# TomClabault/RayTracerCPP

Measured on NVIDIA B200. Metric: Mrays/s (primary+shadow), higher is better.
Workload: dtype f32

## Files before the change

### include/rtb200.h

```cpp
#ifndef RTB200_H
#define RTB200_H

#include <stddef.h>
#include <stdint.h>

#ifdef __cplusplus
extern "C" {
#endif

typedef struct RtContext RtContext;

typedef enum RtStatus {
    RT_OK = 0,
    RT_ERR_INVALID = -1,
    RT_ERR_CUDA = -2,
    RT_ERR_STATE = -3,
    RT_ERR_UNSUPPORTED = -4
} RtStatus;

typedef struct RtMaterial {
    float ambient_coeff[3];
    float diffuse[3];
    float specular[3];
    float emission[3];
// ... 44 lines not shown
    float ssao_amount;
    int32_t enable_clipping;
} RtSettings;

enum {
    RT_TEX_AO = 0,
    RT_TEX_DIFFUSE = 1,
    RT_TEX_NORMAL = 2,
    RT_TEX_ROUGHNESS = 3,
    RT_TEX_SKYSPHERE = 4,
    RT_TEX_SKYBOX_RIGHT = 5,
    RT_TEX_SKYBOX_LEFT = 6,
    RT_TEX_SKYBOX_TOP = 7,
    RT_TEX_SKYBOX_BOTTOM = 8,
    RT_TEX_SKYBOX_BACK = 9,
    RT_TEX_SKYBOX_FRONT = 10,
    RT_TEX_DISPLACEMENT = 11,
    RT_TEX_COUNT = 12
};

typedef struct RtRenderStats {
    uint64_t primary_rays;
    uint64_t shadow_rays;
    uint64_t reflection_rays;
    uint64_t reflection_shadow_rays;
    uint64_t primary_hits;
    uint32_t kernel_launches;
    float    device_ms;
    float    trace_primary_ms;
    float    shade_ms;
    float    reflect_ms;
    float    compact_ms;
    float    resolve_ms;
    uint64_t primary_volume_tests, primary_triangle_tests;
    uint64_t shadow_volume_tests, shadow_triangle_tests;
    uint64_t reflection_volume_tests, reflection_triangle_tests;
    uint64_t traced_primary_rays;
    uint64_t primary_fetched_bytes, shadow_fetched_bytes, reflection_fetched_bytes;
} RtRenderStats;

typedef struct RtBvhInfo {
    uint64_t triangles;
    uint64_t nodes;
    uint64_t leaves;
    uint64_t empty_leaves;
    uint64_t interior;
    uint32_t max_depth_reached;
    uint32_t max_leaf_size;
    uint64_t child_records;
    uint64_t device_bytes;
    double   build_ms;
    double   upload_ms;
} RtBvhInfo;

void rt_default_settings(RtSettings* s);
uint32_t rt_pixel_seed(uint32_t pixel_index, uint32_t rng_seed);

int rt_create(int device, RtContext** out);
void rt_destroy(RtContext* ctx);
const char* rt_last_error(const RtContext* ctx);

enum {
    RT_OPT_COUNT_WORK = 0,
    RT_OPT_CHUNK_PIXELS = 1,
    RT_OPT_REFILL_PRIMARY = 3,
    RT_OPT_REFILL_SHADE = 4,
    RT_OPT_TRI_BATCH = 5,
    RT_OPT_PACKETS = 6,
    RT_OPT_PACKET_ROUNDS = 7,
    RT_OPT_PRIMARY_ROUNDS = 11,
    RT_OPT_ITEM_ROUNDS = 10,
    RT_OPT_ITEM_PASSES = 16,
    RT_OPT_FUSED_ITEMS = 12,
    RT_OPT_TOP_TABLE = 13,
    RT_OPT_DEVICE_BUILD = 15,
    RT_OPT_SHADOW_SORT = 14,
    RT_OPT_SCREEN_CULL = 8,
    RT_OPT_LANES = 9,
    RT_OPT_PACKET_CULL = 19,
    RT_OPT_FAN_LANES = 20,
    RT_OPT_GRAPH = 18,
    RT_OPT_RASTER_UNITS = 17,
    RT_OPT_LIGHT_CULL = 21,
    RT_OPT_LEAF_SPLIT = 2
};
int rt_set_option(RtContext* ctx, int option, int64_t value);
int rt_set_host_threads(int n);
int rt_set_stream(RtContext* ctx, void* cuda_stream);

int rt_set_triangles(RtContext* ctx, const float* xyz9, const float* uv6, const int32_t* mat, size_t n);

int rt_build_bvh(RtContext* ctx, int max_depth, int leaf_max_obj_count);
int rt_bvh_info(const RtContext* ctx, RtBvhInfo* out);

int rt_transform_triangles(RtContext* ctx, const float m[16], int max_depth, int leaf_max_obj_count);

typedef struct RtObjMesh RtObjMesh;
int rt_obj_load(const char* path, const float transform[16], int32_t current_material_count, RtObjMesh** out, char* err, size_t err_cap);
void rt_obj_free(RtObjMesh* mesh);
size_t rt_obj_triangle_count(const RtObjMesh* mesh);
size_t rt_obj_material_count(const RtObjMesh* mesh);
const float* rt_obj_xyz9(const RtObjMesh* mesh);
const float* rt_obj_uv6(const RtObjMesh* mesh);
const int32_t* rt_obj_material_indices(const RtObjMesh* mesh);
const RtMaterial* rt_obj_materials(const RtObjMesh* mesh);
const char* rt_obj_material_name(const RtObjMesh* mesh, size_t i);
void rt_precompute_materials(RtMaterial* mats, size_t n);

int rt_set_materials(RtContext* ctx, const RtMaterial* mats, size_t n);

int rt_add_sphere(RtContext* ctx, const float center[3], float radius, int32_t mat_index);
int rt_add_plane(RtContext* ctx, const float point[3], const float normal[3], int32_t mat_index);
int rt_clear_analytic_shapes(RtContext* ctx);

int rt_set_texture_f32(RtContext* ctx, int slot, const float* rgba, int width, int height);
int rt_set_texture_u8(RtContext* ctx, int slot, const uint8_t* rgba, int width, int height);
int rt_clear_texture(RtContext* ctx, int slot);

int rt_set_camera(RtContext* ctx, const float proj_inv[16], const float cam_to_world[16], const float position[3]);
void rt_perspective_inverse(float fov, float aspect, float znear, float zfar, float proj_inv_out[16]);
void rt_invert_transform(const float m[16], float out[16]);
void rt_transform_point(const float m[16], const float p[3], float out[3]);

int rt_set_projection(RtContext* ctx, float fov, float aspect, float znear, float zfar);

int rt_set_light(RtContext* ctx, const float position[3]);

int rt_render(RtContext* ctx, const RtSettings* settings, uint32_t* argb_out, RtRenderStats* stats);

int rt_render_device(RtContext* ctx, const RtSettings* settings, uint32_t* d_argb_out,
                     int tile_size, int tile_mod, int tile_rem, RtRenderStats* stats);

int rt_render_device_begin(RtContext* ctx, const RtSettings* settings, uint32_t* d_argb_out,
                           int tile_size, int tile_mod, int tile_rem);
int rt_render_device_end(RtContext* ctx, RtRenderStats* stats);

#define RT_FRAME_HANDLE_BYTES 64
int rt_frame_alloc(RtContext* ctx, size_t bytes, void** d_ptr_out, unsigned char handle_out[RT_FRAME_HANDLE_BYTES]);
int rt_frame_open(RtContext* ctx, const unsigned char handle[RT_FRAME_HANDLE_BYTES], void** d_ptr_out);
int rt_frame_close(RtContext* ctx, void* d_ptr);
int rt_frame_free(RtContext* ctx, void* d_ptr);

int rt_frame_to_host(RtContext* ctx, const uint32_t* d_frame, uint32_t* host_out, size_t n_pixels);

int rt_tile_count(const RtSettings* settings, int tile_size, int tile_mod, int tile_rem);
int rt_pack_tiles(RtContext* ctx, const RtSettings* settings, const uint32_t* d_frame, uint32_t* d_staging,
                  int tile_size, int tile_mod, int tile_rem);
int rt_unpack_tiles(RtContext* ctx, const RtSettings* settings, uint32_t* d_frame, const uint32_t* d_staging,
                    int tile_size, int tile_mod, int tile_rem);

int rt_unpack_gathered(RtContext* ctx, const RtSettings* settings, uint32_t* d_frame, const uint32_t* d_gathered,
                       int tile_size, int tile_mod, int self_rem);

int rt_intersect(RtContext* ctx, const float* o3, const float* d3, size_t n,
                 int32_t* tri_id, float* t, float* u, float* v);

int rt_occluded(RtContext* ctx, const float* p3, const float* n3, size_t n, uint8_t* occluded);

int rt_generate_primary_rays(RtContext* ctx, const RtSettings* settings, float* o3, float* d3);

int rt_resolve_ssaa(RtContext* ctx, const uint32_t* argb_in, int width, int height, int factor, uint32_t* argb_out);

#ifdef __cplusplus
}
#endif
#endif
// ... 1 lines not shown
```

### raytracercpp_b200/api.py

```python
from __future__ import annotations

import ctypes as C
from pathlib import Path

import numpy as np

PKG = Path(__file__).resolve().parent
LIB_PATH = PKG / "librtb200.so"

RT_OK, RT_ERR_INVALID, RT_ERR_CUDA, RT_ERR_STATE, RT_ERR_UNSUPPORTED = 0, -1, -2, -3, -4
RT_SHADING, RT_ABS_NORMALS_SHADING, RT_PASTEL_NORMALS_SHADING, RT_BARYCENTRIC_COORDINATES_SHADING, RT_VISUALIZE_AO = range(5)
RT_TEX_AO, RT_TEX_DIFFUSE, RT_TEX_NORMAL, RT_TEX_ROUGHNESS, RT_TEX_SKYSPHERE = range(5)
RT_TEX_SKYBOX_RIGHT, RT_TEX_SKYBOX_LEFT, RT_TEX_SKYBOX_TOP, RT_TEX_SKYBOX_BOTTOM, RT_TEX_SKYBOX_BACK, RT_TEX_SKYBOX_FRONT = range(5, 11)
RT_TEX_DISPLACEMENT = 11
RT_OPT_COUNT_WORK, RT_OPT_CHUNK_PIXELS, RT_OPT_LEAF_SPLIT, RT_OPT_REFILL_PRIMARY, RT_OPT_REFILL_SHADE, RT_OPT_TRI_BATCH, RT_OPT_PACKETS = 0, 1, 2, 3, 4, 5, 6
RT_OPT_PACKET_ROUNDS, RT_OPT_SCREEN_CULL, RT_OPT_LANES, RT_OPT_ITEM_ROUNDS, RT_OPT_PRIMARY_ROUNDS, RT_OPT_FUSED_ITEMS, RT_OPT_TOP_TABLE, RT_OPT_SHADOW_SORT, RT_OPT_DEVICE_BUILD, RT_OPT_ITEM_PASSES = 7, 8, 9, 10, 11, 12, 13, 14, 15, 16
RT_OPT_RASTER_UNITS, RT_OPT_GRAPH, RT_OPT_PACKET_CULL, RT_OPT_FAN_LANES, RT_OPT_LIGHT_CULL = 17, 18, 19, 20, 21


class RtError(RuntimeError):
    def __init__(self, code: int, message: str):
        super().__init__(f"rtb200 error {code}: {message}")
        self.code = code
        self.message = message


class RtMaterial(C.Structure):
    _fields_ = [("ambient_coeff", C.c_float * 3), ("diffuse", C.c_float * 3), ("specular", C.c_float * 3),
                ("emission", C.c_float * 3), ("reflection", C.c_float), ("roughness", C.c_float), ("ns", C.c_float),
                ("specular_threshold", C.c_float)]


SETTINGS_FIELDS = [
    "image_width", "image_height", "enable_ssaa", "ssaa_factor", "hybrid_rasterization_tracing", "shading_method",
    "compute_shadows", "max_recursion_depth", "enable_bvh", "bvh_max_depth", "bvh_leaf_object_count", "enable_ssao",
    "enable_ambient", "enable_diffuse", "enable_specular", "enable_emissive", "rough_reflections_sample_count",
    "enable_ao_mapping", "enable_diffuse_mapping", "enable_normal_mapping", "enable_displacement_mapping",
    "enable_roughness_mapping", "enable_skysphere", "enable_skybox",
]


class RtSettings(C.Structure):
    _fields_ = [(n, C.c_int32) for n in SETTINGS_FIELDS] + [("rng_seed", C.c_uint32), ("displacement_mapping_strength", C.c_float),
                                                              ("parallax_mapping_steps", C.c_int32),
                                                              ("ssao_sample_count", C.c_int32), ("ssao_radius", C.c_float), ("ssao_amount", C.c_float),
                                                             ("enable_clipping", C.c_int32)]

    def copy(self) -> "RtSettings":
        out = RtSettings()
        C.memmove(C.byref(out), C.byref(self), C.sizeof(RtSettings))
        return out


class RtRenderStats(C.Structure):
    _fields_ = [("primary_rays", C.c_uint64), ("shadow_rays", C.c_uint64), ("reflection_rays", C.c_uint64),
                ("reflection_shadow_rays", C.c_uint64), ("primary_hits", C.c_uint64), ("kernel_launches", C.c_uint32),
                ("device_ms", C.c_float), ("trace_primary_ms", C.c_float), ("shade_ms", C.c_float),
                ("reflect_ms", C.c_float), ("compact_ms", C.c_float), ("resolve_ms", C.c_float),
                ("primary_volume_tests", C.c_uint64), ("primary_triangle_tests", C.c_uint64),
                ("shadow_volume_tests", C.c_uint64), ("shadow_triangle_tests", C.c_uint64),
                ("reflection_volume_tests", C.c_uint64), ("reflection_triangle_tests", C.c_uint64),
                ("traced_primary_rays", C.c_uint64), ("primary_fetched_bytes", C.c_uint64), ("shadow_fetched_bytes", C.c_uint64),
                ("reflection_fetched_bytes", C.c_uint64)]

    def as_dict(self) -> dict:
        return {n: getattr(self, n) for n, _ in self._fields_}

    @property
    def total_rays(self) -> int:
        return self.primary_rays + self.shadow_rays + self.reflection_rays + self.reflection_shadow_rays

    @property
    def traced_rays(self) -> int:
        return self.traced_primary_rays + self.shadow_rays + self.reflection_rays + self.reflection_shadow_rays

    @property
    def work_bytes(self) -> int:
        v = self.primary_volume_tests + self.shadow_volume_tests + self.reflection_volume_tests
        t = self.primary_triangle_tests + self.shadow_triangle_tests + self.reflection_triangle_tests
        return 56 * v + 36 * t


class RtBvhInfo(C.Structure):
    _fields_ = [("triangles", C.c_uint64), ("nodes", C.c_uint64), ("leaves", C.c_uint64), ("empty_leaves", C.c_uint64),
                ("interior", C.c_uint64), ("max_depth_reached", C.c_uint32), ("max_leaf_size", C.c_uint32),
                ("child_records", C.c_uint64), ("device_bytes", C.c_uint64), ("build_ms", C.c_double),
                ("upload_ms", C.c_double)]

    def as_dict(self) -> dict:
        return {n: getattr(self, n) for n, _ in self._fields_}


FP, IP, UP, BP = C.POINTER(C.c_float), C.POINTER(C.c_int32), C.POINTER(C.c_uint32), C.POINTER(C.c_uint8)

ABI = {
    "rt_default_settings": (None, [C.POINTER(RtSettings)]),
    "rt_pixel_seed": (C.c_uint32, [C.c_uint32, C.c_uint32]),
    "rt_create": (C.c_int, [C.c_int, C.POINTER(C.c_void_p)]),
    "rt_destroy": (None, [C.c_void_p]),
    "rt_last_error": (C.c_char_p, [C.c_void_p]),
# ... 315 lines not shown
```

### raytracercpp_b200/build.py

```python
from __future__ import annotations

import os
import shutil
import subprocess
import sys
from pathlib import Path

PKG = Path(__file__).resolve().parent
CSRC = PKG / "csrc"
LIB = PKG / "librtb200.so"
SOURCES = [CSRC / "rtb200.cu", CSRC / "octree_build.cpp", CSRC / "scene_io.cpp"]
HEADERS = [CSRC / "kernels.cuh", CSRC / "octree_device.cuh", CSRC / "light_cull.cuh", CSRC / "host_common.h", CSRC / "rt_device.h", CSRC / "rt_math.h", CSRC / "scene_layout.h",
           CSRC / "ssao.cuh", CSRC / "ssao_device.h", CSRC / "raster.cuh", CSRC / "raster_device.h",
           PKG.parent / "include" / "rtb200.h"]

NVCC_FLAGS = [
    "-gencode", "arch=compute_100a,code=sm_100a",
    "-O3", "-lineinfo", "-std=c++17",
    "--fmad=false", "--prec-div=true", "--prec-sqrt=true",
    "-Xcompiler", "-fPIC,-fopenmp,-ffp-contract=off,-O3",
    "-ccbin", "/usr/bin/g++",
    "-shared", "-lgomp",
]


def nvcc() -> str:
    for cand in (os.environ.get("NVCC"), shutil.which("nvcc"), "/usr/local/cuda/bin/nvcc"):
        if cand and Path(cand).exists():
            return cand
    raise RuntimeError("nvcc not found")


def up_to_date() -> bool:
    if not LIB.exists():
        return False
    t = LIB.stat().st_mtime
    return all(p.stat().st_mtime <= t for p in SOURCES + HEADERS + [Path(__file__)])


def build(force: bool = False, verbose: bool = False, extra=(), out: Path | None = None) -> Path:
    if out is None and not force and up_to_date():
        return LIB
    cmd = [nvcc(), *NVCC_FLAGS, *extra, "-o", str(out or LIB), *map(str, SOURCES)]
    if verbose:
        print(" ".join(cmd), flush=True)
    res = subprocess.run(cmd, capture_output=True, text=True)
    if verbose or res.returncode:
        sys.stderr.write(res.stdout + res.stderr)
    if res.returncode:
        raise RuntimeError("nvcc failed")
    return out or LIB


if __name__ == "__main__":
    argv = sys.argv[1:]
    out = Path(argv[argv.index("--out") + 1]) if "--out" in argv else None
    extra = [a for a in argv if a.startswith("-D")] + (["-Xptxas", "-v"] if "--ptxas" in argv else [])
    print(build(force="--force" in argv, verbose=True, extra=extra, out=out))
```

### raytracercpp_b200/csrc/kernels.cuh

```cuda
#pragma once

#include <cuda_runtime.h>
#include "rt_device.h"

namespace rtb {

constexpr int kPatch = 8;
constexpr int kPrimaryThreads = 128;
constexpr int kQueueThreads = 128;
constexpr int kPrimaryFetch = 1;
constexpr int kStepsPerCheck = 4;
constexpr unsigned kParkCtas = 296;
constexpr unsigned kFusedGenerations = 12;
constexpr int kItemPasses = 6;
#ifndef RTB_SHADE_MINB
#define RTB_SHADE_MINB 7
#endif

constexpr int kSubQueues = 32;
struct alignas(128) SubQueue {
    unsigned int n;
    unsigned int next;
    unsigned int pad[30];
};
struct alignas(16) FusedTotals {
    unsigned int reserved;
    unsigned int done;
    unsigned int packets_done;
    unsigned int pad;
};

struct ChunkCounters {
    unsigned int next_patch;
    unsigned int next_shade;
    unsigned int n_hits;
    unsigned int n_refl;
    unsigned int stack_overflow;
    unsigned int n_split;
    unsigned int items_n[kItemPasses];
    unsigned int items_next[kItemPasses];
    unsigned int p_split, p_items_n[kItemPasses], p_items_next[kItemPasses];
    SubQueue sq[2][kSubQueues];
    FusedTotals ft[2];
    unsigned long long refl_rays;
    unsigned long long refl_shadow_rays;
    unsigned long long primary_vol, primary_tri, shadow_vol, shadow_tri, refl_vol, refl_tri;
    unsigned long long primary_fetch, shadow_fetch, refl_fetch;
    unsigned long long traced_primary;
    unsigned int rounds_hist[2][16];
    unsigned int max_rounds[2];
    unsigned long long max_packet_ns[2], sum_packet_ns[2];
};

RT_DEV unsigned long long global_ns()
{
    unsigned long long t;
    asm volatile("mov.u64 %0, %%globaltimer;" : "=l"(t));
    return t;
}

RT_DEV void note_packet(ChunkCounters* cnt, int which, unsigned rounds, unsigned long long ns)
{
    const int b = rounds ? min(31 - __clz(rounds), 15) : 0;
    atomicAdd(&cnt->rounds_hist[which][b], 1u);
    atomicMax(&cnt->max_rounds[which], rounds);
    atomicMax(&cnt->max_packet_ns[which], ns);
    atomicAdd(&cnt->sum_packet_ns[which], ns);
}

RT_DEV void flush_work(TraceCounters& tc, unsigned long long* vol, unsigned long long* tri, unsigned long long* fetch)
{
    unsigned long long v = tc.vol_tests, t = tc.tri_tests, f = 64ull * tc.rec_fetch + 48ull * tc.tri_fetch;
#pragma unroll
    for (int o = 16; o > 0; o >>= 1) {
        v += __shfl_xor_sync(0xffffffffu, v, o);
        t += __shfl_xor_sync(0xffffffffu, t, o);
        f += __shfl_xor_sync(0xffffffffu, f, o);
    }
    if ((threadIdx.x & 31u) == 0) {
        if (v) atomicAdd(vol, v);
        if (t) atomicAdd(tri, t);
        if (f) atomicAdd(fetch, f);
    }
}

struct WorkView {
    const uint32_t* tiles;
    uint32_t tile_begin, tile_end;
    int32_t tiles_x;
    int32_t tile_px;
    int32_t patches_per_side;
    const uint32_t* cover;
    int32_t cover_words;
};

struct QueueView {
    int32_t* slot_tri;
    float* slot_t;
    float* slot_u;
    float* slot_v;
    uint32_t* hit_slot;
    uint32_t* hit_sorted;
    uint32_t sort_mode, sort_slots;
    float* g_z;
    V3* g_n;
    uint32_t* split_base;
    uint32_t* split_active;
    uint32_t* split_occ;
    uint4* items;
    uint32_t split_capacity, item_capacity;
    uint32_t* item_ready;
    uint32_t* split_pending;
    uint32_t tag;
    unsigned long long* split_best;
    uint32_t* refl_idx;
    float* refl_rgb;
    unsigned long long* refl_cnt;
    uint32_t capacity;
};

RT_DEV bool slot_pixel(const WorkView& wk, const FrameView& fr, uint32_t slot, int& px, int& py)
{
    const uint32_t pps = (uint32_t)wk.patches_per_side;
    const uint32_t per_tile = pps * pps * (uint32_t)(kPatch * kPatch);
    const uint32_t tile = wk.tiles[wk.tile_begin + slot / per_tile];
    const uint32_t in_tile = slot % per_tile;
    const uint32_t patch = in_tile / (uint32_t)(kPatch * kPatch), in_patch = in_tile % (uint32_t)(kPatch * kPatch);
    const int lx = (int)(patch % pps) * kPatch + (int)(in_patch & 7u);
    const int ly = (int)(patch / pps) * kPatch + (int)(in_patch >> 3);
    px = (int)(tile % (uint32_t)wk.tiles_x) * wk.tile_px + lx;
    py = (int)(tile / (uint32_t)wk.tiles_x) * wk.tile_px + ly;
    return lx < wk.tile_px && ly < wk.tile_px && px < fr.rw && py < fr.rh;
}

RT_DEV bool covered(const WorkView& wk, int px, int py)
{
    if (wk.cover == nullptr) return true;
    const uint32_t w = __ldg(wk.cover + ((uint32_t)py >> 2) * (uint32_t)wk.cover_words + ((uint32_t)px >> 8));
    return ((w >> (((uint32_t)px >> 3) & 31u)) & 1u) != 0u;
}

struct Tuning {
    int32_t primary_refill;
    int32_t shade_refill;
    int32_t tri_batch;
    int32_t packets;
    int32_t packet_rounds;
    int32_t item_rounds;
    int32_t primary_rounds;
    int32_t fused;
    int32_t packet_min, item_min, primary_min;
    int32_t item_passes;
    int32_t cull;
};

struct Drain {
    const unsigned int* counter;
    uint32_t total;
    int min_rounds;
};
RT_DEV Drain no_drain() { Drain d; d.counter = nullptr; d.total = 0u; d.min_rounds = 0; return d; }
RT_DEV Drain make_drain(const unsigned int* counter, uint32_t total, int min_rounds)
{
    Drain d; d.counter = min_rounds > 0 ? counter : nullptr; d.total = total; d.min_rounds = min_rounds; return d;
}

template <bool ANY, bool COUNT>
RT_DEV void warp_step(const SceneView& sc, RayState& S, RayStack& K, TraceCounters* tc, bool alive, const Tuning& tune)
{
    const unsigned want_c = __ballot_sync(0xffffffffu, alive && S.mode == RT_MODE_CHILDREN);
    const unsigned want_t = __ballot_sync(0xffffffffu, alive && S.mode == RT_MODE_TRIANGLES);
    if (want_c != 0u && __popc(want_t) < tune.tri_batch) {
        if (alive && S.mode == RT_MODE_CHILDREN) ray_child_step<COUNT>(sc, S, K, tc);
    } else if (want_t != 0u) {
        if (alive && S.mode == RT_MODE_TRIANGLES) ray_triangle_step<ANY, COUNT>(sc, S, K, tc);
    }
}
// ... 141 lines not shown
    const float2 q1b = *(reinterpret_cast<const float2*>(rec + 1) + 1);
    const float4 q2 = rec[2], q3 = rec[3];
    RT_SLAB(3, q1b.x, q1b.y)
    RT_SLAB(4, q2.x, q2.y)
    RT_SLAB(5, q2.z, q2.w)
    RT_SLAB(6, q3.x, q3.y)
#undef RT_SLAB
    link = f4_bits(q3.z); meta = f4_bits(q3.w);
    const bool ok = pass && (tn <= tf + 2.0f * sr.slack) && (tf + sr.slack >= 0.0f) && (tn - sr.slack <= t_limit);
    return ok ? tn - sr.slack : INFINITY;
}

RT_DEV uint32_t ld_vol(const unsigned int* p) { return *((const volatile unsigned int*)p); }

template <bool ORDERED, bool COUNT>
RT_DEV bool packet_cell(const float4* rec, uint32_t count, const SlabRay& sr, float t_max, bool active, PacketStack& K, int& sp, TraceCounters& tc,
                        uint32_t keep)
{
    const unsigned lane = threadIdx.x & 31u;
    const int base = sp;
    for (uint32_t m = keep; m != 0u; m &= m - 1u) {
        const uint32_t k = (uint32_t)__ffs((int)m) - 1u;
        if (COUNT && active) tc.vol_tests++;
        uint32_t cl = 0u, cm = 0u;
        const float tn = slab_entry_packet<ORDERED>(rec + 4 * k, sr, t_max, active, cl, cm);
        if (__ballot_sync(0xffffffffu, tn != INFINITY) == 0u) continue;
        const float tmin = warp_min(tn);
        if (sp >= RT_STACK_SIZE) return false;
        if (lane == 0) {
            int j = sp;
            while (j > base && K.t[j - 1] < tmin) {
                K.t[j] = K.t[j - 1]; K.link[j] = K.link[j - 1]; K.meta[j] = K.meta[j - 1];
                --j;
            }
            K.t[j] = tmin; K.link[j] = cl; K.meta[j] = cm;
        }
        ++sp;
    }
    return true;
}

struct TopTable {
    float4 rec[4 * RT_TOP_RECORDS];
    unsigned long long bar;
};
struct NoTopTable {
    unsigned long long bar;
};
template <bool TOP> struct TopStorage { typedef TopTable type; };
template <> struct TopStorage<false> { typedef NoTopTable type; };
RT_DEV const float4* top_pointer(TopTable& T) { return T.rec; }
RT_DEV const float4* top_pointer(NoTopTable&) { return nullptr; }
RT_DEV void load_top_table(const SceneView&, NoTopTable&) {}

RT_DEV void load_top_table(const SceneView& sc, TopTable& T)
{
    const uint32_t bar = (uint32_t)__cvta_generic_to_shared(&T.bar), dst = (uint32_t)__cvta_generic_to_shared(&T.rec[0]);
    const uint32_t bytes = (uint32_t)sc.top_n * 64u;
    if (bytes == 0u) return;
    if (threadIdx.x == 0) {
        asm volatile("mbarrier.init.shared::cta.b64 [%0], 1;" ::"r"(bar));
        asm volatile("fence.mbarrier_init.release.cluster;" ::: "memory");
    }
    __syncthreads();
    if (threadIdx.x == 0) {
        asm volatile("mbarrier.arrive.expect_tx.shared::cta.b64 _, [%0], %1;" ::"r"(bar), "r"(bytes) : "memory");
        asm volatile("cp.async.bulk.shared::cluster.global.mbarrier::complete_tx::bytes [%0], [%1], %2, [%3];" ::"r"(dst), "l"(sc.top), "r"(bytes), "r"(bar)
                     : "memory");
    }
    asm volatile(
        "{\n"
        ".reg .pred p;\n"
        "TOP_WAIT:\n"
        "mbarrier.try_wait.parity.shared::cta.b64 p, [%0], 0;\n"
        "@!p bra TOP_WAIT;\n"
        "}\n" ::"r"(bar)
        : "memory");
}

template <bool ANY, bool COUNT, bool CULL = false>
RT_DEV bool packet_trace(const SceneView& sc, PacketStack& K, const float4* top, bool& active, V3 o, V3 d, float t_max, V3 p, float dist2,
                         HitRec& best, bool& occluded, TraceCounters& tc, unsigned& overflow, int max_rounds, unsigned& rounds,
                         uint32_t start_link = 0u, uint32_t start_meta = 0u, int32_t best_orig = 0x7fffffff,
                         const unsigned int* poll_occ = nullptr, const unsigned long long* poll_best = nullptr, Drain drain = no_drain())
{
    const unsigned lane = threadIdx.x & 31u;
    SlabRay sr;
    slab_setup(o, d, sr);
    const V3 md = -d;
    best.tri = -1; best.t = -1.0f; best.u = 1.0f; best.v = 0.0f;
    occluded = false;
    unsigned neg_mask = 0u;
#ifdef RTB_NO_ORDERED
    bool ordered = false;
#else
    bool ordered = true;
#endif
#pragma unroll
    for (int i = 0; i < 7; i++) {
        const bool nz = active && sr.inv[i] != 0.0f;
        const unsigned bn = __ballot_sync(0xffffffffu, nz && sr.inv[i] < 0.0f), bp = __ballot_sync(0xffffffffu, nz && sr.inv[i] > 0.0f);
        if (bn != 0u && bp != 0u) ordered = false;
        if (bn != 0u) neg_mask |= 1u << i;
    }
    const unsigned f = lane & 3u;
    const bool swap_lo = ordered && ((neg_mask >> (2u * f)) & 1u) != 0u;
    const bool swap_hi = ordered && f < 3u && ((neg_mask >> (2u * f + 1u)) & 1u) != 0u;
    uint32_t link = start_link, meta = start_meta;
    if (start_meta == 0u) {
        const rt_f4* r = sc.recs;
        rt_f4 q0 = RT_LDG4(r), q1 = RT_LDG4(r + 1), q2 = RT_LDG4(r + 2), q3 = RT_LDG4(r + 3);
        if (COUNT && active) tc.vol_tests++;
        if (COUNT && lane == 0) tc.rec_fetch++;
        const float tn = active ? slab_entry(q0, q1, q2, q3, sr, t_max) : INFINITY;
        link = f4_bits(q3.z); meta = f4_bits(q3.w);
        if (__ballot_sync(0xffffffffu, tn != INFINITY) == 0u || (meta & ~(RT_LEAF_BIT | RT_META_TOP)) == 0u) return true;
        if (ANY && (__ldg(sc.blk_occ) & 1u) == 0u) return true;
    }
    int sp = 0;
    for (;;) {
        if (max_rounds > 0 && sp < RT_STACK_SIZE) {
            bool stop = (int)rounds >= max_rounds;
            if (!stop && drain.counter != nullptr && (int)rounds >= drain.min_rounds && (rounds & 15u) == 0u) {
                uint32_t handed = 0;
                if (lane == 0) handed = ld_vol(drain.counter);
                stop = __shfl_sync(0xffffffffu, handed, 0) >= drain.total;
            }
            if (stop) {
                if (lane == 0) { K.t[sp] = 0.0f; K.link[sp] = link; K.meta[sp] = meta; K.saved = sp + 1; }
                __syncwarp();
                return false;
            }
        }
        ++rounds;
        if ((rounds & 3u) == 0u) {
            if (ANY && poll_occ != nullptr) {
                uint32_t w = 0;
                if (lane == 0) w = ld_vol(poll_occ);
                w = __shfl_sync(0xffffffffu, w, 0);
                if ((w >> lane) & 1u) active = false;
                if (__ballot_sync(0xffffffffu, active) == 0u) return true;
            }
            if (!ANY && poll_best != nullptr) {
                const unsigned long long key = *((const volatile unsigned long long*)(poll_best + lane));
                if (key != ~0ull) {
                    const float te = __uint_as_float((uint32_t)(key >> 32));
                    const int32_t oe = (int32_t)(uint32_t)key;
                    if (te < t_max || (te == t_max && oe < best_orig)) { t_max = te; best_orig = oe; }
                }
            }
        }
        if (!(meta & RT_LEAF_BIT)) {
            const uint32_t count = meta & RT_META_COUNT_MASK;
            const bool in_top = top != nullptr && (meta & RT_META_TOP) != 0u;
            if (lane < 4u * count) {
                float4 v = in_top ? top[4u * ((meta >> RT_META_TOP_SHIFT) & 0xffu) + lane] : RT_LDG4(sc.recs + 4 * (size_t)link + lane);
                if (swap_lo) { const float t = v.x; v.x = v.y; v.y = t; }
                if (swap_hi) { const float t = v.z; v.z = v.w; v.w = t; }
                K.stage[lane] = v;
            }
            if (COUNT && lane == 0 && !in_top) tc.rec_fetch += count;
            __syncwarp();
            uint32_t keep = (1u << count) - 1u;
            if (ANY) keep &= __ldg(sc.blk_occ + (link >> 1));
            if (CULL) {
                const uint32_t child = lane >> 2;
                const float4 pl = K.plane[lane & 3u];
                const float4 b0 = K.stage[4u * child];
                const float2 b1 = *reinterpret_cast<const float2*>(&K.stage[4u * child + 1u]);
                const float ax = pl.x * (pl.x > 0.0f ? fmaxf(b0.x, b0.y) : fminf(b0.x, b0.y));
                const float ay = pl.y * (pl.y > 0.0f ? fmaxf(b0.z, b0.w) : fminf(b0.z, b0.w));
                const float az = pl.z * (pl.z > 0.0f ? fmaxf(b1.x, b1.y) : fminf(b1.x, b1.y));
                const bool outside = (ax + ay + az) - pl.w < -4.0e-6f * (fabsf(ax) + fabsf(ay) + fabsf(az) + fabsf(pl.w));
                unsigned m = __ballot_sync(0xffffffffu, outside);
                m |= m >> 1;
                m |= m >> 2;
                unsigned in = ~m & 0x11111111u;
                in = (in | (in >> 3)) & 0x03030303u;
                in = (in | (in >> 6)) & 0x000f000fu;
                in = (in | (in >> 12)) & 0xffu;
                keep &= in;
            }
            const bool fits = ordered ? packet_cell<true, COUNT>(K.stage, count, sr, t_max, active, K, sp, tc, keep)
                                      : packet_cell<false, COUNT>(K.stage, count, sr, t_max, active, K, sp, tc, keep);
            if (!fits) { overflow = 1u; return true; }
            __syncwarp();
        } else {
            const uint32_t cnt = meta & ~RT_LEAF_BIT;
            const uint32_t per_round = CULL ? 8u : 10u;
            for (uint32_t first = 0; first < cnt; first += per_round) {
                const uint32_t m = min(per_round, cnt - first);
                uint32_t keep = (1u << m) - 1u;
                if (ANY) {
                    const uint32_t at = link + first;
                    keep &= __funnelshift_r(__ldg(sc.tri_occ + (at >> 5)), __ldg(sc.tri_occ + (at >> 5) + 1), at & 31u);
                    if (keep == 0u) continue;
                }
                if (lane < 3u * m) K.stage[lane] = RT_LDG4(sc.tris + 3 * (size_t)(link + first) + lane);
                if (COUNT && lane == 0) tc.tri_fetch += m;
                __syncwarp();
                if (CULL) {
                    const uint32_t tri = lane >> 2;
                    const float4 pl = K.plane[lane & 3u];
                    const float4 va = K.stage[3u * tri], vb = K.stage[3u * tri + 1u], vc = K.stage[3u * tri + 2u];
                    const float da = (pl.x * va.x + pl.y * va.y + pl.z * va.z) - pl.w;
                    const float db = (pl.x * vb.x + pl.y * vb.y + pl.z * vb.z) - pl.w;
                    const float dc = (pl.x * vc.x + pl.y * vc.y + pl.z * vc.z) - pl.w;
                    const float mag = fabsf(pl.w) + fmaxf(fabsf(va.x), fmaxf(fabsf(vb.x), fabsf(vc.x))) + fmaxf(fabsf(va.y), fmaxf(fabsf(vb.y), fabsf(vc.y))) +
                                      fmaxf(fabsf(va.z), fmaxf(fabsf(vb.z), fabsf(vc.z)));
                    const bool outside = fmaxf(da, fmaxf(db, dc)) < -4.0e-6f * mag;
                    unsigned om = __ballot_sync(0xffffffffu, outside);
                    om |= om >> 1;
                    om |= om >> 2;
                    unsigned in = ~om & 0x11111111u;
                    in = (in | (in >> 3)) & 0x03030303u;
                    in = (in | (in >> 6)) & 0x000f000fu;
                    in = (in | (in >> 12)) & 0xffu;
                    keep &= in;
                }
                for (uint32_t km = keep; km != 0u; km &= km - 1u) {
                    const uint32_t i = (uint32_t)__ffs((int)km) - 1u;
                    const float4 p0 = K.stage[3 * i], p1 = K.stage[3 * i + 1], p2 = K.stage[3 * i + 2];
                    if (COUNT && active) tc.tri_tests++;
                    float t, u, v;
                    if (active && tri_test(p0, p1, p2, o, md, t, u, v)) {
                        const uint32_t tri = link + first + i;
                        if (ANY) {
                            if (t > 0.0f) {
                                V3 q = o + t * d;
                                if (length2(p - q) < dist2) { occluded = true; active = false; }
                            }
                        } else if (t < t_max || (t == t_max && sc.orig[tri] < best_orig)) {
                            t_max = t;
                            best_orig = sc.orig[tri];
                            best.tri = (int32_t)tri; best.t = t; best.u = u; best.v = v;
                        }
                    }
                }
                __syncwarp();
            }
            if (ANY && __ballot_sync(0xffffffffu, active) == 0u) return true;
        }
        bool got = false;
        while (sp > 0) {
            --sp;
            const float et = K.t[sp];
            if (__ballot_sync(0xffffffffu, active && et <= t_max) == 0u) continue;
            link = K.link[sp]; meta = K.meta[sp];
            got = true;
            break;
        }
        if (!got) return true;
    }
}

RT_DEV bool emit_items(const QueueView& q, unsigned int* items_n, const PacketStack& K, int pass, uint32_t sidx)
{
    const unsigned lane = threadIdx.x & 31u;
    const uint32_t n = (uint32_t)K.saved;
    uint32_t at = 0;
    if (lane == 0) at = atomicAdd(&items_n[pass], n);
    at = __shfl_sync(0xffffffffu, at, 0);
    const bool ok = at + n <= q.item_capacity;
    uint4* region = q.items + (size_t)pass * q.item_capacity;
    for (uint32_t i = lane; i < n && at + i < q.item_capacity; i += 32u)
        region[at + i] = ok ? make_uint4(sidx, K.link[i], K.meta[i], 0u) : make_uint4(0xffffffffu, 0u, 0u, 0u);
    __syncwarp();
    return ok;
}

RT_DEV unsigned long long closest_key(float t, int32_t orig) { return ((unsigned long long)__float_as_uint(t) << 32) | (uint32_t)orig; }
constexpr unsigned long long kNoHitKey = ~0ull;

#ifndef RTB_PRIMARY_MINB
#define RTB_PRIMARY_MINB 8
#endif
#define RTB_PRIMARY_BOUNDS __launch_bounds__(kPrimaryThreads, RTB_PRIMARY_MINB)
template <bool COUNT, bool TOP>
__global__ void RTB_PRIMARY_BOUNDS
k_primary_packet(SceneView sc, FrameView fr, WorkView wk, QueueView q, ChunkCounters* cnt, uint32_t* super, Tuning tune)
{
    __shared__ PacketStack stacks[kPrimaryThreads / 32];
    PacketStack& K = stacks[threadIdx.x >> 5];
    __shared__ typename TopStorage<TOP>::type top_table;
    load_top_table(sc, top_table);
    const float4* top = top_pointer(top_table);
    const unsigned lane = threadIdx.x & 31u;
    const uint32_t pps = (uint32_t)wk.patches_per_side;
    const uint32_t total = (wk.tile_end - wk.tile_begin) * pps * pps * (uint32_t)(kPatch * kPatch);
    TraceCounters tc = zero_counters();
    unsigned overflow = 0;
    uint32_t traced = 0;
    uint32_t nxt = 0;
    if (lane == 0) nxt = atomicAdd(&cnt->next_patch, 32u * kPrimaryFetch);
    for (;;) {
        const uint32_t first = __shfl_sync(0xffffffffu, nxt, 0);
        if (first >= total) break;
        if (lane == 0) nxt = atomicAdd(&cnt->next_patch, 32u * kPrimaryFetch);
#pragma unroll 1
        for (uint32_t b = 0; b < (uint32_t)kPrimaryFetch; b++) {
            const uint32_t base = first + 32u * b;
            if (base >= total) break;
            const uint32_t slot = base + lane;
            int px = 0, py = 0;
            const bool active = slot < total && slot_pixel(wk, fr, slot, px, py);
            V3 o = v3(0, 0, 0), d = v3(0, 0, 1);
            const bool inside = active && covered(wk, px, py);
            if (__ballot_sync(0xffffffffu, inside) == 0u) {
                if (slot < total) {
                    q.slot_tri[slot] = -1;
                    if (active) {
                        if (miss_needs_ray(fr)) primary_ray(fr, px, py, o, d);
                        super[(size_t)py * fr.rw + px] = quantise_argb(shade_miss(sc, fr, d));
                    }
                }
                continue;
            }
            if (active) primary_ray(fr, px, py, o, d);
            traced += (uint32_t)__popc(__ballot_sync(0xffffffffu, active));
            HitRec best;
            bool occ, live = active;
            unsigned rounds = 0;
            const unsigned long long t0 = COUNT ? global_ns() : 0ull;
            if (!((tune.cull & 1) != 0 && packet_set_cull(K, active, o, o + d, 0.0f))) packet_no_cull(K);
            const bool finished = packet_trace<false, COUNT, true>(sc, K, top, live, o, d, INFINITY, o, 0.0f, best, occ, tc, overflow, tune.primary_rounds, rounds,
                                                                   0u, 0u, 0x7fffffff, nullptr, nullptr, make_drain(&cnt->next_patch, total, tune.primary_min));
            __syncwarp();
            if (COUNT && lane == 0) note_packet(cnt, 0, rounds, global_ns() - t0);
            if (!finished) {
                const unsigned am = __ballot_sync(0xffffffffu, active);
                uint32_t sidx = 0;
                if (lane == 0) sidx = atomicAdd(&cnt->p_split, 1u);
                sidx = __shfl_sync(0xffffffffu, sidx, 0);
                if (sidx < q.split_capacity && emit_items(q, cnt->p_items_n, K, 0, sidx)) {
                    if (lane == 0) { q.split_base[sidx] = base; q.split_active[sidx] = am; }
                    q.split_best[(size_t)sidx * 32u + lane] = (active && best.tri >= 0) ? closest_key(best.t, sc.orig[best.tri]) : kNoHitKey;
                    continue;
                }
                if (sidx < q.split_capacity && lane == 0) { q.split_base[sidx] = base; q.split_active[sidx] = 0u; }
                live = active;
                packet_trace<false, COUNT>(sc, K, top, live, o, d, INFINITY, o, 0.0f, best, occ, tc, overflow, 0, rounds);
                __syncwarp();
            }
            if (slot < total) {
                const bool hit = active && best.tri >= 0 && best.t > 0.1f;
                q.slot_tri[slot] = hit ? best.tri : -1;
                if (hit) { q.slot_t[slot] = best.t; q.slot_u[slot] = best.u; q.slot_v[slot] = best.v; }
                else if (active) {
                    if (sc.n_shapes > 0) q.slot_t[slot] = (best.tri >= 0 && best.t > 0.0f) ? best.t : -1.0f;
                    super[(size_t)py * fr.rw + px] = quantise_argb(shade_miss(sc, fr, d));
                }
            }
        }
    }
    if (overflow) atomicOr(&cnt->stack_overflow, 1u);
    if (lane == 0 && traced) atomicAdd(&cnt->traced_primary, (unsigned long long)traced);
    if (COUNT) flush_work(tc, &cnt->primary_vol, &cnt->primary_tri, &cnt->primary_fetch);
}

template <bool COUNT>
__global__ void RTB_PRIMARY_BOUNDS
k_primary_items(SceneView sc, FrameView fr, WorkView wk, QueueView q, ChunkCounters* cnt, Tuning tune, int pass)
{
    __shared__ PacketStack stacks[kPrimaryThreads / 32];
    PacketStack& K = stacks[threadIdx.x >> 5];
    const float4* top = nullptr;
    const unsigned lane = threadIdx.x & 31u;
    const uint32_t n = min(cnt->p_items_n[pass], q.item_capacity);
    const uint4* region = q.items + (size_t)pass * q.item_capacity;
    const int budget = pass + 1 < tune.item_passes ? tune.item_rounds : 0;
    TraceCounters tc = zero_counters();
    unsigned overflow = 0;
    for (;;) {
        uint32_t i = 0;
        if (lane == 0) i = atomicAdd(&cnt->p_items_next[pass], 1u);
        i = __shfl_sync(0xffffffffu, i, 0);
        if (i >= n) break;
        const uint4 item = region[i];
        const uint32_t sidx = item.x;
        if (sidx == 0xffffffffu) continue;
        const uint32_t base = q.split_base[sidx];
        const uint32_t slot = base + lane;
        const bool active = ((q.split_active[sidx] >> lane) & 1u) != 0u;
        int px = 0, py = 0;
        V3 o = v3(0, 0, 0), d = v3(0, 0, 1);
        if (active) { slot_pixel(wk, fr, slot, px, py); primary_ray(fr, px, py, o, d); }
        unsigned long long* mine = q.split_best + (size_t)sidx * 32u + lane;
        const unsigned long long seen = *((volatile unsigned long long*)mine);
        const float t_start = seen == kNoHitKey ? INFINITY : __uint_as_float((uint32_t)(seen >> 32));
        const int32_t orig_start = seen == kNoHitKey ? 0x7fffffff : (int32_t)(uint32_t)seen;
        HitRec best;
        bool occ, live = active;
        unsigned rounds = 0;
        if (!((tune.cull & 1) != 0 && packet_set_cull(K, active, o, o + d, 0.0f))) packet_no_cull(K);
        bool finished = packet_trace<false, COUNT, true>(sc, K, top, live, o, d, t_start, o, 0.0f, best, occ, tc, overflow, budget, rounds, item.y, item.z, orig_start,
                                                         nullptr, nullptr, make_drain(&cnt->p_items_next[pass], n, tune.item_min));
        __syncwarp();
        if (active && best.tri >= 0) atomicMin(mine, closest_key(best.t, sc.orig[best.tri]));
        if (!finished && !emit_items(q, cnt->p_items_n, K, pass + 1, sidx)) {
            const unsigned long long now = *((volatile unsigned long long*)mine);
            const float t2 = now == kNoHitKey ? INFINITY : __uint_as_float((uint32_t)(now >> 32));
            const int32_t o2 = now == kNoHitKey ? 0x7fffffff : (int32_t)(uint32_t)now;
            live = active;
            packet_trace<false, COUNT>(sc, K, top, live, o, d, t2, o, 0.0f, best, occ, tc, overflow, 0, rounds, item.y, item.z, o2);
            __syncwarp();
            if (active && best.tri >= 0) atomicMin(mine, closest_key(best.t, sc.orig[best.tri]));
        }
    }
    if (overflow) atomicOr(&cnt->stack_overflow, 1u);
// ... 1027 lines not shown
    if (active && best.tri >= 0) atomicMin(mine, closest_key(best.t, sc.orig[best.tri]));
    if (!finished && !fq_emit(q, cnt, 0, K, sidx, item.w + 1u, false)) {
        const unsigned long long now = *((volatile unsigned long long*)mine);
        const float t2 = now == kNoHitKey ? INFINITY : __uint_as_float((uint32_t)(now >> 32));
        const int32_t o2 = now == kNoHitKey ? 0x7fffffff : (int32_t)(uint32_t)now;
        live = active;
        packet_trace<false, COUNT>(sc, K, top, live, o, d, t2, o, 0.0f, best, occ, tc, overflow, 0, rounds, item.y, item.z, o2, nullptr,
                                   q.split_best + (size_t)sidx * 32u);
        __syncwarp();
        if (active && best.tri >= 0) atomicMin(mine, closest_key(best.t, sc.orig[best.tri]));
    }
    __threadfence();
    __syncwarp();
    uint32_t left = 0;
    if (lane == 0) left = atomicSub(&q.split_pending[sidx], 1u);
    left = __shfl_sync(0xffffffffu, left, 0);
    if (left == 1u) {
        __threadfence();
        primary_finish_record(sc, fr, wk, q, super, sidx, total);
    }
    if (lane == 0) { __threadfence(); atomicAdd(&cnt->ft[0].done, 1u); }
}

template <bool COUNT>
__global__ void RTB_PRIMARY_BOUNDS
k_primary_fused(SceneView sc, FrameView fr, WorkView wk, QueueView q, ChunkCounters* cnt, uint32_t* super, Tuning tune)
{
    __shared__ PacketStack stacks[kPrimaryThreads / 32];
    PacketStack& K = stacks[threadIdx.x >> 5];
    const float4* top = nullptr;
    const unsigned lane = threadIdx.x & 31u;
    const uint32_t pps = (uint32_t)wk.patches_per_side;
    const uint32_t total = (wk.tile_end - wk.tile_begin) * pps * pps * (uint32_t)(kPatch * kPatch);
    const uint32_t total_packets = total >> 5;
    TraceCounters tc = zero_counters();
    unsigned overflow = 0;
    uint32_t traced = 0;
    uint32_t nxt = 0;
    if (lane == 0) nxt = atomicAdd(&cnt->next_patch, 32u);
    bool more = true;
    uint32_t my_packets = 0;
    unsigned backoff = 250u;
    const uint32_t per_round = 32u * gridDim.x * (kPrimaryThreads / 32);
    uint32_t rem = total / per_round;
    for (;;) {
        uint4 item;
        const int got = tune.primary_rounds > 0 ? fq_take(q, cnt, 0, !more, item) : 0;
        if (got == 1) {
            primary_item_fused<COUNT>(sc, fr, wk, q, cnt, super, fq_budget(tune.item_rounds, more ? rem : 0u), K, top, item, total, tc, overflow);
            backoff = 250u;
            continue;
        }
        if (!more) {
            if (got == 2) continue;
            if (tune.primary_rounds <= 0 || blockIdx.x >= kParkCtas) break;
            bool done = false;
            if (lane == 0) done = fq_all_done(&cnt->ft[0], total_packets);
            if (__shfl_sync(0xffffffffu, done ? 1 : 0, 0)) break;
            __nanosleep(backoff);
            backoff = min(backoff * 2u, 4000u);
            continue;
        }
        const uint32_t base = __shfl_sync(0xffffffffu, nxt, 0);
        if (base >= total) {
            more = false;
            if (lane == 0 && my_packets && tune.primary_rounds > 0) { __threadfence(); atomicAdd(&cnt->ft[0].packets_done, my_packets); }
            continue;
        }
        if (lane == 0) nxt = atomicAdd(&cnt->next_patch, 32u);
        rem = (total - base) / per_round;
        const uint32_t slot = base + lane;
        int px = 0, py = 0;
        const bool active = slot_pixel(wk, fr, slot, px, py);
        V3 o = v3(0, 0, 0), d = v3(0, 0, 1);
        const bool inside = active && covered(wk, px, py);
        bool deferred = false;
        if (__ballot_sync(0xffffffffu, inside) == 0u) {
            q.slot_tri[slot] = -1;
            if (active) {
                if (miss_needs_ray(fr)) primary_ray(fr, px, py, o, d);
                super[(size_t)py * fr.rw + px] = quantise_argb(shade_miss(sc, fr, d));
            }
        } else {
            if (active) primary_ray(fr, px, py, o, d);
            traced += (uint32_t)__popc(__ballot_sync(0xffffffffu, active));
            HitRec best;
            bool occ, live = active;
            unsigned rounds = 0;
            const unsigned long long t0 = COUNT ? global_ns() : 0ull;
            const bool finished = packet_trace<false, COUNT>(sc, K, top, live, o, d, INFINITY, o, 0.0f, best, occ, tc, overflow,
                                                             fq_budget(tune.primary_rounds, rem), rounds);
            __syncwarp();
            if (COUNT && lane == 0) note_packet(cnt, 0, rounds, global_ns() - t0);
            if (!finished) {
                const unsigned am = __ballot_sync(0xffffffffu, active);
                uint32_t sidx = 0xffffffffu;
                if (lane == 0) sidx = atomicAdd(&cnt->p_split, 1u);
                sidx = __shfl_sync(0xffffffffu, sidx, 0);
                if (sidx < q.split_capacity) {
                    if (lane == 0) { q.split_base[sidx] = base; q.split_active[sidx] = am; }
                    q.split_best[(size_t)sidx * 32u + lane] = (active && best.tri >= 0) ? closest_key(best.t, sc.orig[best.tri]) : kNoHitKey;
                    __threadfence();
                    __syncwarp();
                    deferred = fq_emit(q, cnt, 0, K, sidx, 0u, true);
                }
                if (!deferred) {
                    live = active;
                    packet_trace<false, COUNT>(sc, K, top, live, o, d, INFINITY, o, 0.0f, best, occ, tc, overflow, 0, rounds);
                    __syncwarp();
                }
            }
            if (!deferred) {
                const bool hit = active && best.tri >= 0 && best.t > 0.1f;
                q.slot_tri[slot] = hit ? best.tri : -1;
                if (hit) { q.slot_t[slot] = best.t; q.slot_u[slot] = best.u; q.slot_v[slot] = best.v; }
                else if (active) {
                    if (sc.n_shapes > 0) q.slot_t[slot] = (best.tri >= 0 && best.t > 0.0f) ? best.t : -1.0f;
                    super[(size_t)py * fr.rw + px] = quantise_argb(shade_miss(sc, fr, d));
                }
            }
        }
        ++my_packets;
    }
    if (overflow) atomicOr(&cnt->stack_overflow, 1u);
    if (lane == 0 && traced) atomicAdd(&cnt->traced_primary, (unsigned long long)traced);
    if (COUNT) flush_work(tc, &cnt->primary_vol, &cnt->primary_tri, &cnt->primary_fetch);
}

__global__ void k_fill_miss(SceneView sc, FrameView fr, WorkView wk, uint32_t* super)
{
    const uint32_t n_tiles = wk.tile_end - wk.tile_begin;
    const uint32_t background = quantise_argb(shade_miss(sc, fr, v3(0, 0, 1)));
    if (!miss_needs_ray(fr) && (wk.tile_px & 3) == 0 && (fr.rw & 3) == 0 && (reinterpret_cast<uintptr_t>(super) & 15u) == 0) {
        const uint32_t groups_per_row = (uint32_t)wk.tile_px >> 2;
        const uint32_t per_tile = groups_per_row * (uint32_t)wk.tile_px;
        const uint4 c4 = make_uint4(background, background, background, background);
        for (uint32_t t = blockIdx.x; t < n_tiles; t += gridDim.x) {
            const uint32_t tile = wk.tiles[wk.tile_begin + t];
            const int x0 = (int)(tile % (uint32_t)wk.tiles_x) * wk.tile_px, y0 = (int)(tile / (uint32_t)wk.tiles_x) * wk.tile_px;
            for (uint32_t g = threadIdx.x; g < per_tile; g += blockDim.x) {
                const int px = x0 + (int)((g % groups_per_row) << 2), py = y0 + (int)(g / groups_per_row);
                if (px < fr.rw && py < fr.rh) *reinterpret_cast<uint4*>(super + (size_t)py * fr.rw + px) = c4;
            }
        }
        return;
    }
    const uint32_t per_tile = (uint32_t)wk.tile_px * (uint32_t)wk.tile_px;
    for (uint32_t t = blockIdx.x; t < n_tiles; t += gridDim.x) {
        const uint32_t tile = wk.tiles[wk.tile_begin + t];
        const int x0 = (int)(tile % (uint32_t)wk.tiles_x) * wk.tile_px, y0 = (int)(tile / (uint32_t)wk.tiles_x) * wk.tile_px;
        for (uint32_t g = threadIdx.x; g < per_tile; g += blockDim.x) {
            const int px = x0 + (int)(g % (uint32_t)wk.tile_px), py = y0 + (int)(g / (uint32_t)wk.tile_px);
            if (px >= fr.rw || py >= fr.rh) continue;
            uint32_t c = background;
            if (miss_needs_ray(fr)) {
                V3 o, d;
                primary_ray(fr, px, py, o, d);
                c = quantise_argb(shade_miss(sc, fr, d));
            }
            super[(size_t)py * fr.rw + px] = c;
        }
    }
}

__global__ void k_resolve(const uint32_t* super, uint32_t* out, WorkView wk, int tile_size, int factor, int width, int height, uint32_t n_box,
                          uint32_t fill)
{
    const uint32_t per_tile = (uint32_t)tile_size * (uint32_t)tile_size;
    const uint64_t total = (uint64_t)(wk.tile_end - wk.tile_begin) * per_tile;
    for (uint64_t g = (uint64_t)blockIdx.x * blockDim.x + threadIdx.x; g < total; g += (uint64_t)gridDim.x * blockDim.x) {
        const uint32_t tpos = wk.tile_begin + (uint32_t)(g / per_tile);
        const uint32_t tile = wk.tiles[tpos];
        const uint32_t in = (uint32_t)(g % per_tile);
        const int x = (int)(tile % (uint32_t)wk.tiles_x) * tile_size + (int)(in % (uint32_t)tile_size);
// ... 99 lines not shown
```

### raytracercpp_b200/csrc/octree_device.cuh

```cuda
#pragma once

#include "scene_layout.h"

namespace rtb {
namespace devbuild {

constexpr int kExtraLevels = 0;
constexpr int kMaxKeyLevels = 21;
constexpr int kSortRounds = 64;
constexpr int kSortUnit = 32 * kSortRounds;
constexpr int kScanItems = 4;
constexpr int kScanBlock = 1024 * kScanItems;

struct Params {
    int32_t max_depth, leaf_max, leaf_split, total_depth;
    float s3;
};

struct Stats {
    unsigned long long interior, nonempty_children;
    unsigned int max_depth, max_leaf;
    unsigned int root_lo[3], root_hi[3];
    unsigned int top_n;
};

constexpr uint32_t kCellLeaf = 0u, kCellRefInterior = 1u, kCellDevInterior = 2u;
struct Cells {
    uint32_t* begin;
    uint32_t* end;
    uint32_t* first_child;
    uint32_t* info;
    float* nr;
    float* fr;
    uint32_t* size;
    uint32_t* rec;
    uint32_t* block;
};

__device__ __forceinline__ unsigned int float_order(float f)
{
    const unsigned int b = __float_as_uint(f);
    return b ^ ((b & 0x80000000u) ? 0xffffffffu : 0x80000000u);
}
__device__ __forceinline__ float order_float(unsigned int k)
{
    return __uint_as_float(k ^ ((k & 0x80000000u) ? 0x80000000u : 0xffffffffu));
}

__global__ void k_ob_init(Stats* st)
{
    st->interior = 0ull; st->nonempty_children = 0ull; st->max_depth = 0u; st->max_leaf = 0u; st->top_n = 0u;
    for (int k = 0; k < 3; k++) { st->root_lo[k] = 0xffffffffu; st->root_hi[k] = 0u; }
}

__global__ void __launch_bounds__(256)
k_ob_centroids(const float* xyz9, uint32_t n, float* centroid, Stats* st)
{
    __shared__ unsigned int s_lo[3], s_hi[3];
    if (threadIdx.x < 3) { s_lo[threadIdx.x] = 0xffffffffu; s_hi[threadIdx.x] = 0u; }
    __syncthreads();
    float lo[3] = {INFINITY, INFINITY, INFINITY}, hi[3] = {-INFINITY, -INFINITY, -INFINITY};
    for (uint32_t i = blockIdx.x * blockDim.x + threadIdx.x; i < n; i += gridDim.x * blockDim.x) {
        const float* p = xyz9 + 9 * (size_t)i;
        for (int k = 0; k < 3; k++) {
            const float a = p[k], b = p[3 + k], c = p[6 + k];
            const float mn = fminf(a, fminf(b, c)), mx = fmaxf(a, fmaxf(b, c));
            centroid[3 * (size_t)i + k] = 0.5f * (mn + mx);
            lo[k] = fminf(lo[k], mn); hi[k] = fmaxf(hi[k], mx);
        }
    }
    for (int k = 0; k < 3; k++) {
        unsigned int l = float_order(lo[k]), h = float_order(hi[k]);
        l = __reduce_min_sync(0xffffffffu, l); h = __reduce_max_sync(0xffffffffu, h);
        if ((threadIdx.x & 31u) == 0) { atomicMin(&s_lo[k], l); atomicMax(&s_hi[k], h); }
    }
    __syncthreads();
    if (threadIdx.x < 3) { atomicMin(&st->root_lo[threadIdx.x], s_lo[threadIdx.x]); atomicMax(&st->root_hi[threadIdx.x], s_hi[threadIdx.x]); }
}

__device__ __forceinline__ int descend(V3& lo, V3& hi, V3 c)
{
    const V3 mid = v3((lo.x + hi.x) / 2, (lo.y + hi.y) / 2, (lo.z + hi.z) / 2);
    const int o = (c.x > mid.x ? 1 : 0) + (c.y > mid.y ? 2 : 0) + (c.z > mid.z ? 4 : 0);
    V3 clo, chi;
    switch (o) {
// ... 456 lines not shown

__device__ __forceinline__ float wb_axis_area(const float4* recs, uint32_t r)
{
    const float4 q0 = recs[4 * (size_t)r], q1 = recs[4 * (size_t)r + 1];
    const float dx = q0.y - q0.x, dy = q0.w - q0.z, dz = q1.y - q1.x;
    return dx * dy + dy * dz + dz * dx;
}

__global__ void __launch_bounds__(256)
k_wb_collapse(const float4* recs, const uint32_t* src, uint32_t lf, uint32_t lc, uint32_t* info, uint32_t* counts, uint32_t* members)
{
    const uint32_t j = blockIdx.x * blockDim.x + threadIdx.x;
    if (j >= lc) return;
    const float4 own = recs[4 * (size_t)src[lf + j] + 3];
    const uint32_t meta = __float_as_uint(own.w);
    if (!wb_interior(meta)) { counts[j] = 0u; info[lf + j] = 0u; return; }
    uint32_t m[8], kids[8], link[8];
    float area[8];
    int n = 0;
    auto put = [&](int at, uint32_t r) {
        const float4 q3 = recs[4 * (size_t)r + 3];
        const uint32_t mm = __float_as_uint(q3.w);
        m[at] = r;
        kids[at] = wb_interior(mm) ? (mm & RT_META_COUNT_MASK) : 0u;
        link[at] = __float_as_uint(q3.z);
        area[at] = kids[at] ? wb_axis_area(recs, r) : 0.0f;
    };
    const uint32_t first = __float_as_uint(own.z), count = meta & RT_META_COUNT_MASK;
    for (uint32_t k = 0; k < count; k++) put(n++, first + k);
    for (;;) {
        int best = -1;
        for (int k = 0; k < n; k++)
            if (kids[k] && n - 1 + (int)kids[k] <= 8 && (best < 0 || area[k] > area[best])) best = k;
        if (best < 0) break;
        const int c = (int)kids[best];
        const uint32_t l = link[best];
        for (int k = n - 1; k > best; k--) {
            m[k + c - 1] = m[k]; kids[k + c - 1] = kids[k]; link[k + c - 1] = link[k]; area[k + c - 1] = area[k];
        }
        for (int k = 0; k < c; k++) put(best + k, l + (uint32_t)k);
        n += c - 1;
    }
    for (int k = 0; k < n; k++) members[8 * (size_t)j + k] = m[k];
    counts[j] = (uint32_t)n;
    info[lf + j] = (uint32_t)n | (kCellRefInterior << 4);
}

__global__ void __launch_bounds__(256)
k_wb_children(Cells C, uint32_t* src, uint32_t lf, uint32_t lc, const uint32_t* counts, const uint32_t* members, uint32_t next_first)
{
    const uint32_t j = blockIdx.x * blockDim.x + threadIdx.x;
    if (j >= lc) return;
    const uint32_t kids = C.info[lf + j] & 15u;
    const uint32_t child = next_first + counts[j];
    C.first_child[lf + j] = kids ? child : 0u;
    for (uint32_t k = 0; k < kids; k++) src[child + k] = members[8 * (size_t)j + k];
}

__global__ void __launch_bounds__(256)
k_wb_size(Cells C, uint32_t lf, uint32_t lc)
{
    const uint32_t j = blockIdx.x * blockDim.x + threadIdx.x;
    if (j >= lc) return;
    const uint32_t node = lf + j, kids = C.info[node] & 15u, first = C.first_child[node];
    uint32_t size = kids ? (kids + 1u) & ~1u : 0u;
    for (uint32_t k = 0; k < kids; k++) size += C.size[first + k];
    C.size[node] = size;
}

__global__ void __launch_bounds__(256)
k_wb_records(const float4* recs, const uint32_t* src, Cells C, uint32_t n_nodes, float4* wrecs)
{
    const uint32_t node = blockIdx.x * blockDim.x + threadIdx.x;
    if (node >= n_nodes) return;
    const float4* s = recs + 4 * (size_t)src[node];
    float4* q = wrecs + 4 * (size_t)C.rec[node];
    float4 q3 = s[3];
    const uint32_t kids = C.info[node] & 15u;
    if (kids) { q3.z = __uint_as_float(C.block[node]); q3.w = __uint_as_float(kids); }
    q[0] = s[0]; q[1] = s[1]; q[2] = s[2]; q[3] = q3;
}

__global__ void __launch_bounds__(256)
k_wb_boxes(const float4* recs, const uint32_t* src, const uint32_t* info, uint32_t n, uint32_t first_kept, float* boxes)
{
    const uint32_t node = blockIdx.x * blockDim.x + threadIdx.x;
    if (node >= n) return;
    const float4 q0 = recs[4 * (size_t)src[node]], q1 = recs[4 * (size_t)src[node] + 1];
    const bool keep = node >= first_kept || (info[node] & 15u) == 0u;
    float* b = boxes + 6 * (size_t)node;
    b[0] = keep ? q0.x : INFINITY; b[1] = keep ? q0.z : INFINITY; b[2] = keep ? q1.x : INFINITY;
    b[3] = keep ? q0.y : -INFINITY; b[4] = keep ? q0.w : -INFINITY; b[5] = keep ? q1.y : -INFINITY;
}

__global__ void __launch_bounds__(256)
k_ob_transform(float* xyz, size_t n_vertices, M4 t)
{
    for (size_t i = (size_t)blockIdx.x * blockDim.x + threadIdx.x; i < n_vertices; i += (size_t)gridDim.x * blockDim.x) {
        const V3 p = xform_point(t, v3(xyz[3 * i], xyz[3 * i + 1], xyz[3 * i + 2]));
        xyz[3 * i] = p.x; xyz[3 * i + 1] = p.y; xyz[3 * i + 2] = p.z;
    }
}

}
}
```

### raytracercpp_b200/csrc/rtb200.cu

```cuda
#include "../../include/rtb200.h"

#include <cuda_runtime.h>
#include <omp.h>
#include <sched.h>

#include <algorithm>
#include <atomic>
#include <chrono>
#include <cmath>
#include <cstdarg>
#include <cstdio>
#include <cstdlib>
#include <cstring>
#include <map>
#include <string>
#include <tuple>
#include <vector>

#include "kernels.cuh"
#include "scene_layout.h"
#include "octree_device.cuh"
#include "light_cull.cuh"
#include "ssao.cuh"
#include "raster.cuh"
#include "host_common.h"

using namespace rtb;

namespace {

constexpr uint64_t kChunkPixels = 1ull << 28;
constexpr int kMaxChunks = 256;
constexpr uint32_t kCoverBoxes = 4096;

thread_local std::string g_create_error;
std::atomic<unsigned long long> g_alloc_generation{0};

double now_ms()
{
    return std::chrono::duration<double, std::milli>(std::chrono::steady_clock::now().time_since_epoch()).count();
}

template <typename T>
struct DevBuf {
    T* p = nullptr;
    size_t n = 0;
    cudaError_t ensure(size_t count)
    {
        if (count <= n) return cudaSuccess;
        if (p) cudaFree(p);
        p = nullptr;
        n = 0;
        cudaError_t e = cudaMalloc((void**)&p, std::max<size_t>(count, 1) * sizeof(T));
        if (e == cudaSuccess) n = count;
        g_alloc_generation++;
        return e;
    }
    void release()
    {
        if (p) cudaFree(p);
        p = nullptr;
        n = 0;
        g_alloc_generation++;
    }
};

struct Texture {
    void* d = nullptr;
    int w = 0, h = 0, format = 0;
};

enum Stage { ST_PRIMARY = 0, ST_COMPACT, ST_REFLECT, ST_SHADE, ST_RESOLVE, ST_COUNT };

struct TimedLaunch {
    int stage;
    cudaEvent_t a, b;
    const char* label;
};

struct TileList {
    uint32_t* d = nullptr;
    uint32_t count = 0;
    int tiles_x = 0;
    std::vector<uint32_t> host;
    uint32_t* d_split = nullptr;
    std::vector<uint32_t> split_host;
    uint32_t n_traced = 0;
    uint64_t split_cover = 0;
    int32_t split_tile_px = 0;
    bool split_valid = false;
    float last_hit_fraction = -1.0f;
};
typedef std::tuple<int, int, int, int, int> TileKey;

}

constexpr int kLanes = 2;
constexpr int kMaxLanes = 6;

struct QueueSet {
    DevBuf<uint32_t> hit_slot, refl_idx, split_base, split_active, split_occ, item_ready, split_pending;
    DevBuf<uint32_t> hit_sorted, sort_keys, sort_bins;
    DevBuf<unsigned long long> split_best, refl_cnt;
    DevBuf<uint4> items;
    DevBuf<int32_t> tri;
    DevBuf<float> t, u, v, refl_rgb;
    void release()
    {
        hit_slot.release(); refl_idx.release(); split_base.release(); split_active.release(); split_occ.release(); split_best.release();
        item_ready.release(); split_pending.release(); hit_sorted.release(); sort_keys.release(); sort_bins.release();
        refl_cnt.release(); items.release(); tri.release(); t.release(); u.release(); v.release(); refl_rgb.release();
    }
};

struct Pending {
    bool active = false;
// ... 29 lines not shown

struct RtContext {
    int device = 0;
    int sm_count = 0;
    cudaStream_t stream = nullptr;
    cudaStream_t own_stream = nullptr;
    std::string error;

    std::vector<float> xyz9, uv6;
    std::vector<int32_t> mat;
    bool has_uv = false, has_mat = false;
    int32_t max_mat_index = -1, min_mat_index = 0;

    bool bvh_valid = false;
    RtBvhInfo info{};
    DevBuf<float4> d_recs, d_tris, d_shade, d_mats, d_top;
    DevBuf<float4> d_wrecs;
    bool wide_tree = false;
    uint64_t n_wrecs = 0;
    uint64_t tree_serial = 0;
    int top_n = 0;
    DevBuf<int32_t> d_orig, d_leaf_of;
    std::vector<HostShape> shapes;
    DevBuf<float4> d_shapes;
    uint32_t n_tris = 0;
    int n_mats = 0;
    bool any_reflective = false;
    Texture tex[RT_TEX_COUNT];

    M4 proj_inv{}, cam_to_world{};
    V3 cam_pos{0, 0, 0};
    V3 light{3, 3, 2};
    bool camera_set = false;

    DevBuf<uint32_t> d_super, d_frame;
    std::map<TileKey, TileList> tile_lists;
    QueueSet qs[kMaxLanes];
    cudaStream_t lane_stream[kMaxLanes] = {nullptr, nullptr, nullptr, nullptr, nullptr, nullptr};
    cudaEvent_t lane_fork = nullptr, lane_join[kMaxLanes] = {nullptr, nullptr, nullptr, nullptr, nullptr, nullptr};
    DevBuf<ChunkCounters> d_counters;
    DevBuf<unsigned int> d_flag;
    std::vector<cudaEvent_t> event_pool;
    size_t events_used = 0;
    std::vector<TimedLaunch> timed;
    size_t stack_limit_set = 0;
    bool opt_count_work = false;
    int opt_leaf_split = 8;
    Tuning tune{16, 16, 8, 1, -256, -16, -256, 0, 0, 0, 0, kItemPasses, 3};
    uint32_t frame_serial = 0;
    uint64_t opt_chunk_pixels = kChunkPixels;
    Pending pending;
    uint32_t* h_frame = nullptr;
    size_t h_frame_cap = 0;
    cudaEvent_t copy_ev[8] = {nullptr, nullptr, nullptr, nullptr, nullptr, nullptr, nullptr, nullptr};
    int grids[2][11] = {{0, 0, 0, 0, 0, 0, 0, 0, 0, 0, 0}, {0, 0, 0, 0, 0, 0, 0, 0, 0, 0, 0}};
    int grid_intersect = 0, grid_occluded = 0, grid_fan = 0;
    bool opt_screen_cull = true;
    int opt_lanes = kLanes;
    bool opt_top_table = false;
    int opt_shadow_sort = 2;
    bool opt_device_build = true;
    DeviceBuild db;
    DevBuf<float> d_gz;
    DevBuf<V3> d_gn;
    DevBuf<int> d_ao;
    DevBuf<unsigned long long> d_rkeys;
    DevBuf<float2> d_rxy;
    DevBuf<RasterUnit> d_runits;
    DevBuf<unsigned int> d_rcount;
    DevBuf<float4> d_rfrag;
    size_t raster_smem_set = 0;
    bool opt_graph = true;
    bool opt_fan_lanes = true;
    bool capturing = false;
    struct FrameGraph { std::string key; cudaGraphExec_t exec; uint32_t launches; };
    std::vector<FrameGraph> graphs;
    std::vector<std::string> seen_keys;
    size_t raster_units0 = (size_t)1 << 18;
    M4 proj{};
    float proj_fov = 45.0f, proj_aspect = 1.0f;
    bool proj_set = false;
    float root_lo[3] = {0, 0, 0}, root_hi[3] = {0, 0, 0};
    std::vector<float> cover_boxes;
    struct CoverInputs { M4 proj_inv, cam_to_world; V3 cam_pos; int32_t rw, rh; uint64_t tree; } cover_in{};
    bool cover_valid = false;
    bool cover_bound = false;
    int32_t cover_words = 0;
    std::vector<uint32_t> h_cover;
    DevBuf<uint32_t> d_cover;
    uint64_t cover_generation = 0;

    bool opt_light_cull = true;
    DevBuf<uint32_t> d_tri_occ, d_blk_occ, d_rec_parent;
    struct LightMaskInputs { V3 light; float span; uint32_t all_set; uint64_t tree; } mask_in{}, mask_next{};
    uint32_t mask_words = 0, mask_recs = 0;
    bool mask_valid = false;
    uint64_t mask_generation = 0;

    DevBuf<float> b_a, b_b, b_t, b_u, b_v;
    DevBuf<int32_t> b_id;
    DevBuf<uint8_t> b_occ;
};

namespace {

int fail(RtContext* ctx, int code, const char* fmt, ...)
{
    char buf[512];
    va_list ap;
    va_start(ap, fmt);
    vsnprintf(buf, sizeof(buf), fmt, ap);
    va_end(ap);
    if (ctx) ctx->error = buf;
    else g_create_error = buf;
    return code;
}

#define RT_CUDA(ctx, expr)                                                                                  \
    do {                                                                                                    \
        cudaError_t e__ = (expr);                                                                           \
        if (e__ != cudaSuccess) return fail(ctx, RT_ERR_CUDA, "%s: %s", #expr, cudaGetErrorString(e__));   \
    } while (0)

int bind(RtContext* ctx)
{
    RT_CUDA(ctx, cudaSetDevice(ctx->device));
    return RT_OK;
}

cudaEvent_t next_event(RtContext* ctx)
{
    if (ctx->events_used == ctx->event_pool.size()) {
        cudaEvent_t e;
        cudaEventCreate(&e);
        ctx->event_pool.push_back(e);
    }
    return ctx->event_pool[ctx->events_used++];
}

struct ScopedTimer {
    RtContext* ctx;
    TimedLaunch tl;
    cudaStream_t stream;
    bool on;
    ScopedTimer(RtContext* c, int stage, cudaStream_t st = nullptr, const char* label = nullptr) : ctx(c), stream(st ? st : c->stream)
    {
        static const bool trace = getenv("RTB200_TRACE") != nullptr;
        on = (label == nullptr || trace) && !c->capturing;
        if (!on) return;
        tl.stage = stage;
        tl.label = label;
        tl.a = next_event(c);
        tl.b = next_event(c);
        cudaEventRecord(tl.a, stream);
    }
    ~ScopedTimer()
    {
        if (!on) return;
        cudaEventRecord(tl.b, stream);
        ctx->timed.push_back(tl);
    }
};

SceneView scene_view(const RtContext* ctx)
{
    SceneView sc;
    memset(&sc, 0, sizeof(sc));
    sc.recs = ctx->d_recs.p;
    sc.top = ctx->d_top.p;
    sc.top_n = ctx->top_n;
    sc.tris = ctx->d_tris.p;
    sc.shade = ctx->d_shade.p;
    sc.mats = ctx->d_mats.p;
// ... 76 lines not shown
    }
    RT_CUDA(ctx, cudaGetLastError());
    ctx->mask_in = in;
    ctx->mask_valid = true;
    return RT_OK;
}

int validate_settings(RtContext* ctx, const RtSettings* s)
{
    std::string why;
    int r = check_settings(s, why);
    return r ? fail(ctx, r, "%s", why.c_str()) : RT_OK;
}

int validate_scene_for_render(RtContext* ctx, const RtSettings* s)
{
    SceneFacts f;
    f.bvh_valid = ctx->bvh_valid; f.camera_set = ctx->camera_set; f.n_tris = ctx->n_tris; f.n_mats = ctx->n_mats;
    f.min_mat_index = ctx->min_mat_index; f.max_mat_index = ctx->max_mat_index;
    for (int i = 0; i < RT_TEX_COUNT; i++) f.tex_format[i] = ctx->tex[i].format;
    f.n_shapes = (int)ctx->shapes.size();
    for (const HostShape& sh : ctx->shapes) {
        const int m = (int)(sh.bits & 0x7fffffffu);
        f.shape_min_mat = std::min(f.shape_min_mat, m);
        f.shape_max_mat = std::max(f.shape_max_mat, m);
    }
    std::string why;
    int r = check_scene_for_render(f, s, why);
    return r ? fail(ctx, r, "%s", why.c_str()) : RT_OK;
}

FrameView frame_view(const RtContext* ctx, const RtSettings* s)
{
    FrameView fr;
    memset(&fr, 0, sizeof(fr));
    fr.proj_inv = ctx->proj_inv;
    fr.cam_to_world = ctx->cam_to_world;
    fr.cam_pos = ctx->cam_pos;
    fr.light = ctx->light;
    fr.factor = s->enable_ssaa ? s->ssaa_factor : 1;
    fr.rw = s->image_width * fr.factor;
    fr.rh = s->image_height * fr.factor;
    fr.s = *s;
    return fr;
}

int check_tile_args(RtContext* ctx, int tile_size, int tile_mod, int tile_rem)
{
    if (tile_size <= 0 || tile_mod <= 0 || tile_rem < 0 || tile_rem >= tile_mod)
        return fail(ctx, RT_ERR_INVALID, "tile_size %d tile_mod %d tile_rem %d", tile_size, tile_mod, tile_rem);
    return RT_OK;
}

int grid_for(const RtContext* ctx, const void* kernel, int threads)
{
    int per_sm = 1;
    cudaOccupancyMaxActiveBlocksPerMultiprocessor(&per_sm, kernel, threads, 0);
    if (per_sm < 1) per_sm = 1;
    return ctx->sm_count * per_sm;
}

bool invert4(const double a[16], double out[16])
{
    double m[4][8];
    for (int i = 0; i < 4; i++)
        for (int j = 0; j < 4; j++) { m[i][j] = a[4 * i + j]; m[i][4 + j] = i == j ? 1.0 : 0.0; }
    for (int c = 0; c < 4; c++) {
        int piv = c;
        for (int r = c + 1; r < 4; r++) if (std::fabs(m[r][c]) > std::fabs(m[piv][c])) piv = r;
        if (std::fabs(m[piv][c]) < 1e-300) return false;
        if (piv != c) for (int j = 0; j < 8; j++) std::swap(m[piv][j], m[c][j]);
        const double d = 1.0 / m[c][c];
        for (int j = 0; j < 8; j++) m[c][j] *= d;
        for (int r = 0; r < 4; r++) {
            if (r == c) continue;
            const double f = m[r][c];
            if (f != 0.0) for (int j = 0; j < 8; j++) m[r][j] -= f * m[c][j];
        }
    }
    for (int i = 0; i < 4; i++) for (int j = 0; j < 4; j++) out[4 * i + j] = m[i][4 + j];
    return true;
}

bool screen_coverage(const M4& cam_to_world, const M4& proj_inv, V3 cam_pos, int rw, int rh, const float* boxes, size_t n_boxes,
                     double margin_scale, std::vector<uint32_t>& bits, int32_t& words_per_row)
{
    const int bw = (rw + 7) / 8, bh = (rh + 3) / 4;
    words_per_row = (bw + 31) / 32;
    bits.assign((size_t)words_per_row * (size_t)bh, 0u);
    auto set_blocks = [&](int bx0, int by0, int bx1, int by1) {
        for (int by = by0; by <= by1; by++) {
            uint32_t* row = bits.data() + (size_t)by * words_per_row;
            for (int w = bx0 >> 5; w <= bx1 >> 5; w++) {
                const int lo = std::max(bx0 - 32 * w, 0), hi = std::min(bx1 - 32 * w, 31);
                row[w] |= (hi == 31 ? 0xffffffffu : ((1u << (hi + 1)) - 1u)) & ~((1u << lo) - 1u);
            }
        }
    };
    if (n_boxes == 0) return true;
    double c2w[16], pinv[16], w2c[16], proj[16];
    for (int i = 0; i < 16; i++) { c2w[i] = (&cam_to_world.m[0][0])[i]; pinv[i] = (&proj_inv.m[0][0])[i]; }
    if (!invert4(c2w, w2c) || !invert4(pinv, proj)) return false;
    const double w0 = c2w[15];
    if (!(std::fabs(w0) > 1e-12)) return false;
    const double centre[3] = {c2w[3] / w0, c2w[7] / w0, c2w[11] / w0};
    const double pos[3] = {cam_pos.x, cam_pos.y, cam_pos.z};
    double scale = 1.0, dc = 0.0;
    for (int k = 0; k < 3; k++) scale = std::max(scale, std::fabs(centre[k]));
    for (int k = 0; k < 3; k++) {
        if (!(std::fabs(centre[k] - pos[k]) <= 1e-5 * scale)) return false;
        dc += (centre[k] - pos[k]) * (centre[k] - pos[k]);
    }
    dc = std::sqrt(dc);
    for (int k = 0; k < 5; k++) {
        const double nx = k == 4 ? 0.0 : (k & 1 ? 1.0 : -1.0), ny = k == 4 ? 0.0 : (k & 2 ? 1.0 : -1.0);
        double v[4];
        for (int i = 0; i < 4; i++) v[i] = pinv[4 * i] * nx + pinv[4 * i + 1] * ny - pinv[4 * i + 2] + pinv[4 * i + 3];
        if (!(std::fabs(v[3]) > 1e-12)) return false;
        for (int i = 0; i < 3; i++) v[i] /= v[3];
        for (const double along : {1.0, 7.5}) {
            const double q[4] = {v[0] * along, v[1] * along, v[2] * along, 1.0};
            double c[4];
            for (int i = 0; i < 4; i++) c[i] = proj[4 * i] * q[0] + proj[4 * i + 1] * q[1] + proj[4 * i + 2] * q[2] + proj[4 * i + 3] * q[3];
            if (!(c[3] > 0.0) || !(std::fabs(c[0] / c[3] - nx) < 1e-4) || !(std::fabs(c[1] / c[3] - ny) < 1e-4)) return false;
        }
    }
    const double eps = 0x1p-24;
    double VS[3] = {0, 0, 0}, WS[3] = {0, 0, 0}, ws_c[4][3], wmin = 1e300, w2min = 1e300, wsign = 0.0, w2sign = 0.0;
    for (int k = 0; k < 4; k++) {
        const double h[4] = {k & 1 ? 1.0 : -1.0, k & 2 ? 1.0 : -1.0, -1.0, 1.0};
        double vh[4], wh[4];
        for (int i = 0; i < 4; i++) vh[i] = pinv[4 * i] * h[0] + pinv[4 * i + 1] * h[1] + pinv[4 * i + 2] * h[2] + pinv[4 * i + 3] * h[3];
        if (k == 0) wsign = vh[3] < 0.0 ? -1.0 : 1.0;
        if (!(vh[3] * wsign > 0.0)) return false;
        wmin = std::min(wmin, std::fabs(vh[3]));
        const double vs[4] = {vh[0] / vh[3], vh[1] / vh[3], vh[2] / vh[3], 1.0};
        for (int i = 0; i < 4; i++) wh[i] = c2w[4 * i] * vs[0] + c2w[4 * i + 1] * vs[1] + c2w[4 * i + 2] * vs[2] + c2w[4 * i + 3];
        if (k == 0) w2sign = wh[3] < 0.0 ? -1.0 : 1.0;
        if (!(wh[3] * w2sign > 0.0)) return false;
        w2min = std::min(w2min, std::fabs(wh[3]));
        for (int i = 0; i < 3; i++) {
            ws_c[k][i] = wh[i] / wh[3];
            VS[i] = std::max(VS[i], std::fabs(vs[i]));
            WS[i] = std::max(WS[i], std::fabs(ws_c[k][i]));
        }
    }
    double e1[4], ev[3], e2[4], e3n = 0.0;
    for (int i = 0; i < 4; i++)
        e1[i] = 6.0 * eps * (std::fabs(pinv[4 * i]) + std::fabs(pinv[4 * i + 1]) + std::fabs(pinv[4 * i + 2]) + std::fabs(pinv[4 * i + 3]));
    if (!(wmin > 2.0 * e1[3])) return false;
    for (int i = 0; i < 3; i++) ev[i] = (e1[i] + VS[i] * e1[3]) / (wmin - e1[3]) + 2.0 * eps * VS[i];
    for (int i = 0; i < 4; i++) {
        double s2 = std::fabs(c2w[4 * i + 3]), p2 = 0.0;
        for (int j = 0; j < 3; j++) { s2 += std::fabs(c2w[4 * i + j]) * VS[j]; p2 += std::fabs(c2w[4 * i + j]) * ev[j]; }
        e2[i] = 4.0 * eps * s2 + p2;
    }
    if (!(w2min > 2.0 * e2[3])) return false;
    for (int i = 0; i < 3; i++) {
        const double ew = (e2[i] + WS[i] * e2[3]) / (w2min - e2[3]) + 2.0 * eps * WS[i];
        const double e3 = ew + eps * (WS[i] + std::fabs(pos[i]));
        e3n += e3 * e3;
    }
    e3n = std::sqrt(e3n);
    double u[3], v[3], n[3];
    for (int i = 0; i < 3; i++) { u[i] = ws_c[1][i] - ws_c[0][i]; v[i] = ws_c[2][i] - ws_c[0][i]; }
    n[0] = u[1] * v[2] - u[2] * v[1]; n[1] = u[2] * v[0] - u[0] * v[2]; n[2] = u[0] * v[1] - u[1] * v[0];
    const double nn = std::sqrt(n[0] * n[0] + n[1] * n[1] + n[2] * n[2]);
    const double lmin = std::fabs(n[0] * (ws_c[0][0] - pos[0]) + n[1] * (ws_c[0][1] - pos[1]) + n[2] * (ws_c[0][2] - pos[2])) / nn;
    if (!(lmin > 4.0 * e3n)) return false;
    const double e_dir = 2.0 * e3n / lmin + 5.0 * eps;
    const double kTriRel = 0x1p-14;
    const double pos_max = std::max(std::fabs(pos[0]), std::max(std::fabs(pos[1]), std::fabs(pos[2])));
    const double ndc_slack = 1e-9;
    for (size_t b = 0; b < n_boxes; b++) {
        const float* bx = boxes + 6 * b;
        bool finite = true, empty = false;
        double lo[3], hi[3], bmax = 0.0;
        for (int k = 0; k < 3; k++) {
            lo[k] = bx[k]; hi[k] = bx[3 + k];
            finite &= std::isfinite(lo[k]) && std::isfinite(hi[k]);
            empty |= lo[k] > hi[k];
            bmax = std::max(bmax, std::max(std::fabs(lo[k]), std::fabs(hi[k])));
        }
        if (empty) continue;
        if (!finite) { set_blocks(0, 0, bw - 1, bh - 1); return true; }
        double sfar = 0.0;
        for (int c = 0; c < 8; c++) {
            double d2 = 0.0;
            for (int k = 0; k < 3; k++) { const double x = ((c >> k) & 1 ? hi[k] : lo[k]) - pos[k]; d2 += x * x; }
            sfar = std::max(sfar, std::sqrt(d2));
        }
        const double e_tri = kTriRel * (pos_max + bmax + sfar);
        const double reach = (sfar + e_tri) * (1.0 + 5.0 * eps);
        const double r = margin_scale * (e_tri + reach * e_dir + dc * (2.0 + reach / lmin));
        double xmin = 1e300, xmax = -1e300, ymin = 1e300, ymax = -1e300;
        bool whole = false;
        for (int c = 0; c < 8 && !whole; c++) {
            const double p[4] = {(c & 1 ? hi[0] + r : lo[0] - r), (c & 2 ? hi[1] + r : lo[1] - r), (c & 4 ? hi[2] + r : lo[2] - r), 1.0};
            double vv[4], cc[4];
            for (int i = 0; i < 4; i++) vv[i] = w2c[4 * i] * p[0] + w2c[4 * i + 1] * p[1] + w2c[4 * i + 2] * p[2] + w2c[4 * i + 3] * p[3];
            if (!(std::fabs(vv[3]) > 1e-12)) { whole = true; break; }
            for (int i = 0; i < 3; i++) vv[i] /= vv[3];
            vv[3] = 1.0;
            for (int i = 0; i < 4; i++) cc[i] = proj[4 * i] * vv[0] + proj[4 * i + 1] * vv[1] + proj[4 * i + 2] * vv[2] + proj[4 * i + 3] * vv[3];
            if (!(cc[3] > 1e-3 * (1.0 + std::fabs(vv[2])))) { whole = true; break; }
            const double nx = cc[0] / cc[3], ny = cc[1] / cc[3];
            if (!std::isfinite(nx) || !std::isfinite(ny)) { whole = true; break; }
            xmin = std::min(xmin, nx); xmax = std::max(xmax, nx); ymin = std::min(ymin, ny); ymax = std::max(ymax, ny);
        }
        if (whole) { set_blocks(0, 0, bw - 1, bh - 1); return true; }
        const double lim = 1e9;
        const double px0 = std::ceil(std::max(-lim, (xmin - ndc_slack + 1.0) * 0.5 * rw - 0.5)), px1 = std::floor(std::min(lim, (xmax + ndc_slack + 1.0) * 0.5 * rw - 0.5));
        const double py0 = std::ceil(std::max(-lim, (ymin - ndc_slack + 1.0) * 0.5 * rh - 0.5)), py1 = std::floor(std::min(lim, (ymax + ndc_slack + 1.0) * 0.5 * rh - 0.5));
        const int x0 = (int)std::max(0.0, px0), x1 = (int)std::min((double)rw - 1, px1);
        const int y0 = (int)std::max(0.0, py0), y1 = (int)std::min((double)rh - 1, py1);
        if (x0 > x1 || y0 > y1) continue;
        set_blocks(x0 >> 3, y0 >> 2, x1 >> 3, y1 >> 2);
    }
    return true;
}

bool cover_any(const std::vector<uint32_t>& bits, int32_t words_per_row, int x0, int y0, int x1, int y1)
{
    const int bx0 = x0 >> 3, bx1 = x1 >> 3;
    for (int by = y0 >> 2; by <= y1 >> 2; by++) {
        const uint32_t* row = bits.data() + (size_t)by * words_per_row;
        for (int w = bx0 >> 5; w <= bx1 >> 5; w++) {
            const int lo = std::max(bx0 - 32 * w, 0), hi = std::min(bx1 - 32 * w, 31);
            if (row[w] & (hi == 31 ? 0xffffffffu : ((1u << (hi + 1)) - 1u)) & ~((1u << lo) - 1u)) return true;
        }
    }
    return false;
}

int update_cover(RtContext* ctx, const FrameView& fr)
{
    RtContext::CoverInputs in;
    memset(&in, 0, sizeof(in));
    in.proj_inv = ctx->proj_inv; in.cam_to_world = ctx->cam_to_world; in.cam_pos = ctx->cam_pos;
    in.rw = fr.rw; in.rh = fr.rh; in.tree = ctx->tree_serial;
    if (ctx->cover_valid && memcmp(&in, &ctx->cover_in, sizeof(in)) == 0) return RT_OK;
    ctx->cover_valid = false;
    const double t0 = now_ms();
    ctx->cover_bound = screen_coverage(ctx->cam_to_world, ctx->proj_inv, ctx->cam_pos, fr.rw, fr.rh, ctx->cover_boxes.data(),
                                       ctx->cover_boxes.size() / 6, 1.0, ctx->h_cover, ctx->cover_words);
    const double t1 = now_ms();
    double t2 = t1;
    if (ctx->cover_bound) {
        RT_CUDA(ctx, cudaStreamSynchronize(ctx->stream));
        t2 = now_ms();
        RT_CUDA(ctx, ctx->d_cover.ensure(ctx->h_cover.size()));
        RT_CUDA(ctx, cudaMemcpyAsync(ctx->d_cover.p, ctx->h_cover.data(), ctx->h_cover.size() * sizeof(uint32_t), cudaMemcpyHostToDevice, ctx->stream));
    }
    static const bool trace = getenv("RTB200_TRACE") != nullptr;
    if (trace) {
        size_t set = 0;
        for (uint32_t w : ctx->h_cover) set += (size_t)__builtin_popcount(w);
        const size_t blocks = (size_t)((fr.rw + 7) / 8) * (size_t)((fr.rh + 3) / 4);
        fprintf(stderr, "[rtb200] screen coverage: %zu boxes, bound %d, %.4f of the blocks covered, build %.3f ms, upload %.3f ms\n",
                ctx->cover_boxes.size() / 6, (int)ctx->cover_bound, ctx->cover_bound ? (double)set / (double)blocks : 1.0, t1 - t0, now_ms() - t2);
    }
    ctx->cover_in = in;
    ctx->cover_valid = true;
    ctx->cover_generation++;
    return RT_OK;
}

int get_tile_list(RtContext* ctx, const RtSettings* s, int tile_size, int tile_mod, int tile_rem, TileList** out)
{
    const TileKey key(s->image_width, s->image_height, tile_size, tile_mod, tile_rem);
    auto it = ctx->tile_lists.find(key);
    if (it == ctx->tile_lists.end()) {
        if (ctx->tile_lists.size() > 64) {
            RT_CUDA(ctx, cudaStreamSynchronize(ctx->stream));
            for (auto& kv : ctx->tile_lists) { cudaFree(kv.second.d); cudaFree(kv.second.d_split); }
            ctx->tile_lists.clear();
        }
        TileList tl;
        if (tile_rem >= 0) tl.host = owned_tiles(s, tile_size, tile_mod, tile_rem, &tl.tiles_x);
        else {
            std::vector<std::vector<uint32_t>> per(tile_mod);
            size_t longest = 0;
            for (int r = 0; r < tile_mod; r++) { per[r] = owned_tiles(s, tile_size, tile_mod, r, &tl.tiles_x); longest = std::max(longest, per[r].size()); }
            tl.host.assign(longest * tile_mod, 0xffffffffu);
            for (int r = 0; r < tile_mod; r++) std::copy(per[r].begin(), per[r].end(), tl.host.begin() + (size_t)r * longest);
        }
        tl.count = (uint32_t)tl.host.size();
        if (tl.count) {
            RT_CUDA(ctx, cudaMalloc((void**)&tl.d, tl.host.size() * sizeof(uint32_t)));
            RT_CUDA(ctx, cudaMemcpy(tl.d, tl.host.data(), tl.host.size() * sizeof(uint32_t), cudaMemcpyHostToDevice));
        }
        it = ctx->tile_lists.emplace(key, std::move(tl)).first;
    }
    *out = &it->second;
    return RT_OK;
}

LightMap make_light_map(const RtContext* ctx)
{
    LightMap lm;
    const V3 c = v3(0.5f * (ctx->root_lo[0] + ctx->root_hi[0]), 0.5f * (ctx->root_lo[1] + ctx->root_hi[1]), 0.5f * (ctx->root_lo[2] + ctx->root_hi[2]));
    const V3 h = v3(0.5f * (ctx->root_hi[0] - ctx->root_lo[0]), 0.5f * (ctx->root_hi[1] - ctx->root_lo[1]), 0.5f * (ctx->root_hi[2] - ctx->root_lo[2]));
    const float radius = std::sqrt(h.x * h.x + h.y * h.y + h.z * h.z);
    V3 z = c - ctx->light;
    const float dist = std::sqrt(z.x * z.x + z.y * z.y + z.z * z.z);
    if (!(dist > 1.0e-20f) || !std::isfinite(dist)) { z = v3(0, 0, 1); }
    else z = v3(z.x / dist, z.y / dist, z.z / dist);
    const V3 up = std::fabs(z.y) < 0.9f ? v3(0, 1, 0) : v3(1, 0, 0);
    V3 x = v3(up.y * z.z - up.z * z.y, up.z * z.x - up.x * z.z, up.x * z.y - up.y * z.x);
    const float xl = std::sqrt(x.x * x.x + x.y * x.y + x.z * x.z);
    x = v3(x.x / xl, x.y / xl, x.z / xl);
    lm.ex = x;
    lm.ey = v3(z.y * x.z - z.z * x.y, z.z * x.x - z.x * x.z, z.x * x.y - z.y * x.x);
    lm.ez = z;
    lm.scale = 0.0f;
    if (std::isfinite(dist) && std::isfinite(radius) && dist > radius * 1.05f && radius > 0.0f) {
        const float tan_half = radius / std::sqrt(dist * dist - radius * radius);
        lm.scale = 1.0f / tan_half;
    }
    return lm;
}


void transform_host_vertices(RtContext* ctx, const M4& t)
{
    const long long n = (long long)(ctx->xyz9.size() / 3);
#pragma omp parallel for schedule(static)
    for (long long i = 0; i < n; i++) {
        V3 p = xform_point(t, v3(ctx->xyz9[3 * i], ctx->xyz9[3 * i + 1], ctx->xyz9[3 * i + 2]));
        ctx->xyz9[3 * i] = p.x; ctx->xyz9[3 * i + 1] = p.y; ctx->xyz9[3 * i + 2] = p.z;
    }
}

void apply_pending_host_transforms(RtContext* ctx)
{
    for (const M4& t : ctx->db.host_pending) transform_host_vertices(ctx, t);
    ctx->db.host_pending.clear();
}

template <typename T>
cudaError_t grow_keep(DevBuf<T>& b, size_t count, size_t keep, cudaStream_t st)
{
    if (count <= b.n) return cudaSuccess;
    T* fresh = nullptr;
    cudaError_t e = cudaMalloc((void**)&fresh, count * sizeof(T));
    if (e != cudaSuccess) return e;
    if (b.p && keep) e = cudaMemcpyAsync(fresh, b.p, keep * sizeof(T), cudaMemcpyDeviceToDevice, st);
    if (e == cudaSuccess) e = cudaStreamSynchronize(st);
    if (b.p) cudaFree(b.p);
    b.p = fresh;
    b.n = count;
    return e;
}

int scan_counts(RtContext* ctx, uint32_t* data, size_t count, uint32_t* total)
{
    using namespace devbuild;
    DeviceBuild& D = ctx->db;
    const cudaStream_t st = ctx->stream;
    const uint32_t blocks = (uint32_t)((count + kScanBlock - 1) / kScanBlock);
    RT_CUDA(ctx, D.sums.ensure(std::max<uint32_t>(blocks, 1)));
    k_scan_sums<<<blocks, 1024, 0, st>>>(data, count, D.sums.p);
    k_scan_top<<<1, 1024, 0, st>>>(D.sums.p, blocks, total);
    k_scan_apply<<<blocks, 1024, 0, st>>>(data, count, D.sums.p);
    return RT_OK;
}

void root_cover_box(RtContext* ctx)
{
    ctx->cover_boxes.assign({ctx->root_lo[0], ctx->root_lo[1], ctx->root_lo[2], ctx->root_hi[0], ctx->root_hi[1], ctx->root_hi[2]});
}

int build_wide_tree(RtContext* ctx, uint64_t n_records)
{
    using namespace devbuild;
    DeviceBuild& D = ctx->db;
    const cudaStream_t st = ctx->stream;
    const size_t cap = (size_t)n_records;
    RT_CUDA(ctx, D.w_src.ensure(cap)); RT_CUDA(ctx, D.c_first.ensure(cap)); RT_CUDA(ctx, D.c_info.ensure(cap)); RT_CUDA(ctx, D.c_size.ensure(cap));
    RT_CUDA(ctx, D.c_rec.ensure(cap)); RT_CUDA(ctx, D.c_block.ensure(cap)); RT_CUDA(ctx, D.stats.ensure(1));
    Cells C;
    memset(&C, 0, sizeof(C));
    C.first_child = D.c_first.p; C.info = D.c_info.p; C.size = D.c_size.p; C.rec = D.c_rec.p; C.block = D.c_block.p;
    {
        const uint32_t zero = 0u, root_block = 2u;
        RT_CUDA(ctx, cudaMemcpyAsync(D.w_src.p, &zero, 4, cudaMemcpyHostToDevice, st));
        RT_CUDA(ctx, cudaMemcpyAsync(C.rec, &zero, 4, cudaMemcpyHostToDevice, st));
        RT_CUDA(ctx, cudaMemcpyAsync(C.block, &root_block, 4, cudaMemcpyHostToDevice, st));
        RT_CUDA(ctx, cudaStreamSynchronize(st));
    }
    const float4* recs = ctx->d_recs.p;
    uint32_t* d_total = (uint32_t*)&D.stats.p->top_n;
    std::vector<uint32_t> level_first{0u}, level_count{1u};
    for (;;) {
        const uint32_t lf = level_first.back(), lc = level_count.back();
        RT_CUDA(ctx, D.counts.ensure(lc));
        RT_CUDA(ctx, D.w_members.ensure(8 * (size_t)lc));
        k_wb_collapse<<<(lc + 255) / 256, 256, 0, st>>>(recs, D.w_src.p, lf, lc, C.info, D.counts.p, D.w_members.p);
        if (int r = scan_counts(ctx, D.counts.p, lc, d_total)) return r;
        uint32_t total = 0;
        RT_CUDA(ctx, cudaMemcpyAsync(&total, d_total, 4, cudaMemcpyDeviceToHost, st));
        RT_CUDA(ctx, cudaStreamSynchronize(st));
        if (total == 0) break;
        if ((size_t)lf + lc + total > cap) return fail(ctx, RT_ERR_STATE, "wide tree: more nodes than child records");
        k_wb_children<<<(lc + 255) / 256, 256, 0, st>>>(C, D.w_src.p, lf, lc, D.counts.p, D.w_members.p, lf + lc);
        level_first.push_back(lf + lc); level_count.push_back(total);
    }
    const uint32_t n_nodes = level_first.back() + level_count.back();
    {
        size_t lv = 0;
        while (lv + 1 < level_first.size() && level_count[lv + 1] <= kCoverBoxes) lv++;
        const uint32_t n_box = level_first[lv] + level_count[lv];
        RT_CUDA(ctx, D.w_boxes.ensure(6 * (size_t)n_box));
        k_wb_boxes<<<(n_box + 255) / 256, 256, 0, st>>>(recs, D.w_src.p, C.info, n_box, level_first[lv], D.w_boxes.p);
        ctx->cover_boxes.resize(6 * (size_t)n_box);
        RT_CUDA(ctx, cudaMemcpyAsync(ctx->cover_boxes.data(), D.w_boxes.p, 6 * (size_t)n_box * sizeof(float), cudaMemcpyDeviceToHost, st));
        RT_CUDA(ctx, cudaStreamSynchronize(st));
    }
    for (int l = (int)level_first.size() - 1; l >= 0; l--)
        k_wb_size<<<(level_count[l] + 255) / 256, 256, 0, st>>>(C, level_first[l], level_count[l]);
    uint32_t root_size = 0;
    RT_CUDA(ctx, cudaMemcpyAsync(&root_size, C.size, 4, cudaMemcpyDeviceToHost, st));
    RT_CUDA(ctx, cudaStreamSynchronize(st));
    const uint64_t n_wide = 2ull + root_size;
    ctx->n_wrecs = n_wide;
    RT_CUDA(ctx, ctx->d_wrecs.ensure(4 * n_wide));
    RT_CUDA(ctx, cudaMemsetAsync(ctx->d_wrecs.p, 0, 4 * n_wide * sizeof(float4), st));
    Params P;
    memset(&P, 0, sizeof(P));
    for (size_t l = 0; l < level_first.size(); l++)
        k_ob_place<<<(level_count[l] + 255) / 256, 256, 0, st>>>(C, level_first[l], level_count[l], P);
    k_wb_records<<<(n_nodes + 255) / 256, 256, 0, st>>>(recs, D.w_src.p, C, n_nodes, (float4*)ctx->d_wrecs.p);
    k_ob_top_table<<<1, 32, 0, st>>>((float4*)ctx->d_wrecs.p, (float4*)ctx->d_top.p, D.stats.p);
    uint32_t top_n = 0;
    RT_CUDA(ctx, cudaMemcpyAsync(&top_n, &D.stats.p->top_n, 4, cudaMemcpyDeviceToHost, st));
    RT_CUDA(ctx, cudaStreamSynchronize(st));
    RT_CUDA(ctx, cudaGetLastError());
    ctx->top_n = (int)top_n;
    ctx->wide_tree = true;
    if (getenv("RTB200_TRACE"))
        fprintf(stderr, "[rtb200] wide tree: %llu records on %zu levels (narrow: %llu)\n", (unsigned long long)n_wide, level_first.size(),
                (unsigned long long)n_records);
    return RT_OK;
}

int build_bvh_device(RtContext* ctx, int max_depth, int leaf_max)
{
    using namespace devbuild;
    DeviceBuild& D = ctx->db;
    const size_t n = ctx->xyz9.size() / 9;
    const cudaStream_t st = ctx->stream;
    RT_CUDA(ctx, cudaStreamSynchronize(st));
    const double t0 = now_ms();
    if (!D.tris_on_device) {
        apply_pending_host_transforms(ctx);
        RT_CUDA(ctx, D.xyz9.ensure(9 * n));
        RT_CUDA(ctx, cudaMemcpyAsync(D.xyz9.p, ctx->xyz9.data(), 9 * n * sizeof(float), cudaMemcpyHostToDevice, st));
        if (ctx->has_uv) { RT_CUDA(ctx, D.uv6.ensure(6 * n)); RT_CUDA(ctx, cudaMemcpyAsync(D.uv6.p, ctx->uv6.data(), 6 * n * sizeof(float), cudaMemcpyHostToDevice, st)); }
        if (ctx->has_mat) { RT_CUDA(ctx, D.mat.ensure(n)); RT_CUDA(ctx, cudaMemcpyAsync(D.mat.p, ctx->mat.data(), n * sizeof(int32_t), cudaMemcpyHostToDevice, st)); }
        RT_CUDA(ctx, cudaStreamSynchronize(st));
        D.tris_on_device = true;
    }
    const double t1 = now_ms();

    Params P;
    P.max_depth = max_depth; P.leaf_max = leaf_max; P.leaf_split = ctx->opt_leaf_split;
    P.total_depth = std::min(kMaxKeyLevels, max_depth + (ctx->opt_leaf_split > 0 ? kExtraLevels : 0));
    P.s3 = std::sqrt(3.0f) / 3;
    const uint32_t n32 = (uint32_t)n;
    const int wide = ctx->sm_count * 8;
    static const bool trace = getenv("RTB200_TRACE") != nullptr;
    double t_phase = t1;
    auto trace_phase = [&](const char* what) {
        if (!trace) return;
        cudaStreamSynchronize(st);
        const double t = now_ms();
        fprintf(stderr, "[rtb200]   device octree: %s %.2f ms\n", what, t - t_phase);
        t_phase = t;
    };
    RT_CUDA(ctx, D.stats.ensure(1)); RT_CUDA(ctx, D.centroid.ensure(3 * n));
    for (int k = 0; k < 2; k++) { RT_CUDA(ctx, D.keys[k].ensure(n)); RT_CUDA(ctx, D.idx[k].ensure(n)); }
    k_ob_init<<<1, 1, 0, st>>>(D.stats.p);
    k_ob_centroids<<<wide, 256, 0, st>>>(D.xyz9.p, n32, D.centroid.p, D.stats.p);
    k_ob_keys<<<wide, 256, 0, st>>>(D.centroid.p, n32, D.stats.p, P, D.keys[0].p, D.idx[0].p);

    const uint32_t n_units = (n32 + kSortUnit - 1) / kSortUnit;
    const size_t n_hist = (size_t)256 * n_units;
    const uint32_t hist_blocks = (uint32_t)((n_hist + kScanBlock - 1) / kScanBlock);
    RT_CUDA(ctx, D.hist.ensure(n_hist));
    int cur = 0;
    const int passes = (3 * P.total_depth + 7) / 8;
    (void)hist_blocks;
    for (int pass = 0; pass < passes; pass++) {
        k_rs_count<<<(n_units + 3) / 4, 128, 0, st>>>(D.keys[cur].p, n32, 8 * pass, n_units, D.hist.p);
        if (int r = scan_counts(ctx, D.hist.p, n_hist, nullptr)) return r;
        k_rs_scatter<<<(n_units + 3) / 4, 128, 0, st>>>(D.keys[cur].p, D.idx[cur].p, n32, 8 * pass, n_units, D.hist.p, D.keys[cur ^ 1].p, D.idx[cur ^ 1].p);
        cur ^= 1;
    }
    const unsigned long long* keys = D.keys[cur].p;
    const uint32_t* idx = D.idx[cur].p;
    trace_phase("keys + sort");

    size_t cap = 0;
    auto cells_view = [&]() {
        Cells C;
        C.begin = D.c_begin.p; C.end = D.c_end.p; C.first_child = D.c_first.p; C.info = D.c_info.p; C.nr = D.c_nr.p; C.fr = D.c_fr.p;
        C.size = D.c_size.p; C.rec = D.c_rec.p; C.block = D.c_block.p;
        return C;
    };
    auto reserve_cells = [&](size_t want, size_t keep) -> int {
        if (want <= cap) return RT_OK;
        const size_t c = std::max(want, cap * 2);
        RT_CUDA(ctx, grow_keep(D.c_begin, c, keep, st)); RT_CUDA(ctx, grow_keep(D.c_end, c, keep, st)); RT_CUDA(ctx, grow_keep(D.c_first, c, keep, st));
        RT_CUDA(ctx, grow_keep(D.c_info, c, keep, st)); RT_CUDA(ctx, grow_keep(D.c_size, c, keep, st)); RT_CUDA(ctx, grow_keep(D.c_rec, c, keep, st));
        RT_CUDA(ctx, grow_keep(D.c_block, c, keep, st)); RT_CUDA(ctx, grow_keep(D.c_nr, 7 * c, 7 * keep, st)); RT_CUDA(ctx, grow_keep(D.c_fr, 7 * c, 7 * keep, st));
// ... 93 lines not shown
{
    size_t want = 4096 + (size_t)(std::max(0, s->max_recursion_depth) + 2) * 3072;
    if (want > ctx->stack_limit_set) {
        RT_CUDA(ctx, cudaDeviceSetLimit(cudaLimitStackSize, want));
        ctx->stack_limit_set = want;
    }
    return RT_OK;
}

}

extern "C" {

void rt_default_settings(RtSettings* s)
{
    if (s) default_settings(s);
}

uint32_t rt_pixel_seed(uint32_t pixel_index, uint32_t rng_seed) { return pixel_seed(pixel_index, rng_seed); }

void rt_perspective_inverse(float fov, float aspect, float znear, float zfar, float proj_inv_out[16])
{
    M4 inv = invert_matrix(perspective_matrix(fov, aspect, znear, zfar));
    memcpy(proj_inv_out, inv.m, sizeof(inv.m));
}

void rt_invert_transform(const float m[16], float out[16])
{
    M4 a;
    memcpy(a.m, m, sizeof(a.m));
    M4 inv = invert_matrix(a);
    memcpy(out, inv.m, sizeof(inv.m));
}

void rt_transform_point(const float m[16], const float p[3], float out[3])
{
    M4 a;
    memcpy(a.m, m, sizeof(a.m));
    V3 q = xform_point(a, v3(p[0], p[1], p[2]));
    out[0] = q.x; out[1] = q.y; out[2] = q.z;
}

int rt_create(int device, RtContext** out)
{
    if (!out) return fail(nullptr, RT_ERR_INVALID, "out is NULL");
    *out = nullptr;
    int count = 0;
    cudaError_t e = cudaGetDeviceCount(&count);
    if (e != cudaSuccess || count == 0)
        return fail(nullptr, RT_ERR_CUDA, "no CUDA device: %s (this library has no CPU path)", cudaGetErrorString(e));
    if (device < 0 || device >= count) return fail(nullptr, RT_ERR_INVALID, "device %d of %d", device, count);
    RtContext* ctx = new RtContext();
    ctx->device = device;
    cudaDeviceProp prop;
    if ((e = cudaSetDevice(device)) != cudaSuccess || (e = cudaGetDeviceProperties(&prop, device)) != cudaSuccess ||
        (e = cudaStreamCreateWithFlags(&ctx->stream, cudaStreamNonBlocking)) != cudaSuccess) {
        delete ctx;
        return fail(nullptr, RT_ERR_CUDA, "device init: %s", cudaGetErrorString(e));
    }
    ctx->own_stream = ctx->stream;
    ctx->sm_count = prop.multiProcessorCount;
    for (int i = 0; i < 4; i++)
        for (int j = 0; j < 4; j++) ctx->cam_to_world.m[i][j] = ctx->proj_inv.m[i][j] = (i == j) ? 1.0f : 0.0f;
    *out = ctx;
    return RT_OK;
}

void rt_destroy(RtContext* ctx)
{
    if (!ctx) return;
    cudaSetDevice(ctx->device);
    cudaStreamSynchronize(ctx->stream);
    ctx->d_recs.release(); ctx->d_wrecs.release(); ctx->d_top.release(); ctx->d_tris.release(); ctx->d_shade.release(); ctx->d_mats.release(); ctx->d_orig.release(); ctx->d_leaf_of.release(); ctx->d_shapes.release();
    for (auto& t : ctx->tex) if (t.d) cudaFree(t.d);
    ctx->d_super.release(); ctx->d_frame.release(); ctx->db.release(); ctx->d_gz.release(); ctx->d_gn.release(); ctx->d_ao.release();
    for (auto& g : ctx->graphs) cudaGraphExecDestroy(g.exec);
    ctx->d_rkeys.release(); ctx->d_rxy.release(); ctx->d_runits.release(); ctx->d_rcount.release(); ctx->d_rfrag.release();
    for (auto& kv : ctx->tile_lists) { cudaFree(kv.second.d); cudaFree(kv.second.d_split); }
    for (auto& qs : ctx->qs) qs.release();
    for (auto st : ctx->lane_stream) if (st) cudaStreamDestroy(st);
    if (ctx->lane_fork) cudaEventDestroy(ctx->lane_fork);
    for (auto e : ctx->lane_join) if (e) cudaEventDestroy(e);
    ctx->d_counters.release(); ctx->d_flag.release();
    ctx->b_a.release(); ctx->b_b.release(); ctx->b_t.release(); ctx->b_u.release(); ctx->b_v.release(); ctx->b_id.release(); ctx->b_occ.release();
    if (ctx->pending.host_cnt) cudaFreeHost(ctx->pending.host_cnt);
    if (ctx->h_frame) cudaFreeHost(ctx->h_frame);
    for (auto e : ctx->copy_ev) if (e) cudaEventDestroy(e);
    for (auto e : ctx->event_pool) cudaEventDestroy(e);
    cudaStreamDestroy(ctx->own_stream);
    delete ctx;
}

const char* rt_last_error(const RtContext* ctx) { return ctx ? ctx->error.c_str() : g_create_error.c_str(); }

int rt_set_option(RtContext* ctx, int option, int64_t value)
{
    if (!ctx) return RT_ERR_INVALID;
    switch (option) {
    case RT_OPT_COUNT_WORK: ctx->opt_count_work = value != 0; return RT_OK;
    case RT_OPT_LEAF_SPLIT:
        if (value < 0 || value > 1024) return fail(ctx, RT_ERR_INVALID, "leaf split %lld", (long long)value);
        ctx->opt_leaf_split = (int)value;
        ctx->bvh_valid = false;
        return RT_OK;
    case RT_OPT_REFILL_PRIMARY:
    case RT_OPT_REFILL_SHADE:
        if (value < 1 || value > 32) return fail(ctx, RT_ERR_INVALID, "refill threshold %lld outside [1,32]", (long long)value);
        (option == RT_OPT_REFILL_PRIMARY ? ctx->tune.primary_refill : ctx->tune.shade_refill) = (int32_t)value;
        return RT_OK;
    case RT_OPT_TRI_BATCH:
        if (value < 1 || value > 32) return fail(ctx, RT_ERR_INVALID, "triangle batch %lld outside [1,32]", (long long)value);
        ctx->tune.tri_batch = (int32_t)value;
        return RT_OK;
    case RT_OPT_PACKETS:
        ctx->tune.packets = value != 0;
        return RT_OK;
    case RT_OPT_PACKET_ROUNDS:
        if (value < -(1 << 30) || value > (1 << 30)) return fail(ctx, RT_ERR_INVALID, "packet rounds %lld", (long long)value);
        ctx->tune.packet_rounds = (int32_t)value;
        return RT_OK;
    case RT_OPT_PRIMARY_ROUNDS:
        if (value < -(1 << 30) || value > (1 << 30)) return fail(ctx, RT_ERR_INVALID, "primary rounds %lld", (long long)value);
        ctx->tune.primary_rounds = (int32_t)value;
        return RT_OK;
    case RT_OPT_ITEM_ROUNDS:
        if (value == 0 || value < -(1 << 30) || value > (1 << 30)) return fail(ctx, RT_ERR_INVALID, "item rounds %lld", (long long)value);
        ctx->tune.item_rounds = (int32_t)value;
        return RT_OK;
    case RT_OPT_FUSED_ITEMS: ctx->tune.fused = value != 0; return RT_OK;
    case RT_OPT_TOP_TABLE: ctx->opt_top_table = value != 0; return RT_OK;
    case RT_OPT_ITEM_PASSES:
        if (value < 1 || value > kItemPasses) return fail(ctx, RT_ERR_INVALID, "item passes %lld outside [1,%d]", (long long)value, kItemPasses);
        ctx->tune.item_passes = (int32_t)value;
        return RT_OK;
    case RT_OPT_DEVICE_BUILD: ctx->opt_device_build = value != 0; return RT_OK;
    case RT_OPT_SHADOW_SORT:
        if (value < 0 || value > 2) return fail(ctx, RT_ERR_INVALID, "shadow sort %lld outside [0,2]", (long long)value);
        ctx->opt_shadow_sort = (int)value;
        return RT_OK;
    case RT_OPT_SCREEN_CULL: ctx->opt_screen_cull = value != 0; return RT_OK;
    case RT_OPT_LANES:
        if (value < 0 || value > kMaxLanes) return fail(ctx, RT_ERR_INVALID, "lanes %lld outside [0,%d]", (long long)value, kMaxLanes);
        ctx->opt_lanes = value == 1 ? kLanes : (int)std::max<int64_t>(value, 1);
        return RT_OK;
    case RT_OPT_GRAPH: ctx->opt_graph = value != 0; return RT_OK;
    case RT_OPT_LIGHT_CULL: ctx->opt_light_cull = value != 0; return RT_OK;
    case RT_OPT_FAN_LANES: ctx->opt_fan_lanes = value != 0; return RT_OK;
    case RT_OPT_PACKET_CULL:
        if (value < 0 || value > 3) return fail(ctx, RT_ERR_INVALID, "packet cull %lld outside [0,3]", (long long)value);
        ctx->tune.cull = (int32_t)value;
        return RT_OK;
    case RT_OPT_RASTER_UNITS:
        if (value < 1 || value > (1ll << 28)) return fail(ctx, RT_ERR_INVALID, "raster unit list of %lld entries outside [1, 2^28]", (long long)value);
        ctx->d_runits.release();
        ctx->raster_units0 = (size_t)value;
        return RT_OK;
    case RT_OPT_CHUNK_PIXELS:
        if (value < 256 || value > (1ll << 31)) return fail(ctx, RT_ERR_INVALID, "chunk of %lld pixels outside [256, 2^31] (ray slots are 32-bit)", (long long)value);
        ctx->opt_chunk_pixels = (uint64_t)value;
        return RT_OK;
    default: return fail(ctx, RT_ERR_INVALID, "unknown option %d", option);
    }
}

int rt_set_stream(RtContext* ctx, void* cuda_stream)
{
    if (!ctx) return RT_ERR_INVALID;
    if (int r = bind(ctx)) return r;
    RT_CUDA(ctx, cudaStreamSynchronize(ctx->stream));
    ctx->stream = cuda_stream ? (cudaStream_t)cuda_stream : ctx->own_stream;
    return RT_OK;
}

int rt_set_triangles(RtContext* ctx, const float* xyz9, const float* uv6, const int32_t* mat, size_t n)
{
    if (!ctx) return RT_ERR_INVALID;
    if (n && !xyz9) return fail(ctx, RT_ERR_INVALID, "xyz9 is NULL");
    if (n > 0x7fffffffu / 3) return fail(ctx, RT_ERR_INVALID, "too many triangles");
    ctx->xyz9.assign(xyz9, xyz9 + 9 * n);
    ctx->has_uv = uv6 != nullptr;
    ctx->has_mat = mat != nullptr;
    if (uv6) ctx->uv6.assign(uv6, uv6 + 6 * n); else ctx->uv6.clear();
    if (mat) ctx->mat.assign(mat, mat + n); else ctx->mat.clear();
    ctx->min_mat_index = n ? (mat ? *std::min_element(mat, mat + n) : -1) : 0;
    ctx->max_mat_index = n ? (mat ? *std::max_element(mat, mat + n) : -1) : -1;
    ctx->bvh_valid = false;
    ctx->db.tris_on_device = false;
    ctx->db.host_pending.clear();
    return RT_OK;
}

int rt_build_bvh(RtContext* ctx, int max_depth, int leaf_max_obj_count)
{
    if (!ctx) return RT_ERR_INVALID;
    if (int r = bind(ctx)) return r;
    if (max_depth < 0 || max_depth > RT_MAX_TREE_DEPTH) return fail(ctx, RT_ERR_INVALID, "max_depth %d outside [0,%d]", max_depth, RT_MAX_TREE_DEPTH);
    if (leaf_max_obj_count < 0) return fail(ctx, RT_ERR_INVALID, "leaf_max_obj_count %d", leaf_max_obj_count);
    const size_t n = ctx->xyz9.size() / 9;
    ctx->bvh_valid = false;
    ctx->wide_tree = false;
    ctx->cover_boxes.clear();
    ctx->tree_serial++;
    if (ctx->opt_device_build && n > 0) return build_bvh_device(ctx, max_depth, leaf_max_obj_count);
    apply_pending_host_transforms(ctx);
    double t0 = now_ms();
    FlatScene flat;
    build_flat_scene(ctx->xyz9.data(), ctx->has_uv ? ctx->uv6.data() : nullptr, ctx->has_mat ? ctx->mat.data() : nullptr, n,
                     max_depth, leaf_max_obj_count, ctx->opt_leaf_split, flat);
    double t1 = now_ms();
    if (flat.n_records >= (1ull << 28)) return fail(ctx, RT_ERR_INVALID, "scene needs %llu child records (limit 2^28)", (unsigned long long)flat.n_records);
    RT_CUDA(ctx, cudaStreamSynchronize(ctx->stream));
    RT_CUDA(ctx, ctx->d_recs.ensure(flat.recs.size()));
    RT_CUDA(ctx, ctx->d_tris.ensure(flat.tris.size()));
    RT_CUDA(ctx, ctx->d_shade.ensure(flat.shade.size()));
    RT_CUDA(ctx, ctx->d_orig.ensure(flat.orig.size()));
    RT_CUDA(ctx, ctx->d_leaf_of.ensure(flat.orig.size()));
    RawVector<int32_t> leaf_of(flat.orig.size());
#pragma omp parallel for schedule(static)
    for (long long i = 0; i < (long long)flat.orig.size(); i++) leaf_of[(size_t)flat.orig[i]] = (int32_t)i;
    RT_CUDA(ctx, cudaMemcpyAsync(ctx->d_recs.p, flat.recs.data(), flat.recs.size() * sizeof(F4), cudaMemcpyHostToDevice, ctx->stream));
    RT_CUDA(ctx, ctx->d_top.ensure(4 * RT_TOP_RECORDS));
    if (!flat.top.empty()) RT_CUDA(ctx, cudaMemcpyAsync(ctx->d_top.p, flat.top.data(), flat.top.size() * sizeof(F4), cudaMemcpyHostToDevice, ctx->stream));
    ctx->top_n = (int)(flat.top.size() / 4);
    if (n) {
        RT_CUDA(ctx, cudaMemcpyAsync(ctx->d_tris.p, flat.tris.data(), flat.tris.size() * sizeof(F4), cudaMemcpyHostToDevice, ctx->stream));
        RT_CUDA(ctx, cudaMemcpyAsync(ctx->d_shade.p, flat.shade.data(), flat.shade.size() * sizeof(F4), cudaMemcpyHostToDevice, ctx->stream));
        RT_CUDA(ctx, cudaMemcpyAsync(ctx->d_orig.p, flat.orig.data(), flat.orig.size() * sizeof(int32_t), cudaMemcpyHostToDevice, ctx->stream));
        RT_CUDA(ctx, cudaMemcpyAsync(ctx->d_leaf_of.p, leaf_of.data(), leaf_of.size() * sizeof(int32_t), cudaMemcpyHostToDevice, ctx->stream));
    }
    RT_CUDA(ctx, cudaStreamSynchronize(ctx->stream));
    double t2 = now_ms();
    if (n && ctx->opt_leaf_split > 0)
        if (int r = build_wide_tree(ctx, flat.n_records)) return r;
    const double wide_ms = now_ms() - t2;
    ctx->n_tris = (uint32_t)n;
    {
        const F4 *q0 = &flat.recs[0], *q1 = &flat.recs[1];
        ctx->root_lo[0] = q0->x; ctx->root_lo[1] = q0->z; ctx->root_lo[2] = q1->x;
        ctx->root_hi[0] = q0->y; ctx->root_hi[1] = q0->w; ctx->root_hi[2] = q1->y;
    }
    if (!ctx->wide_tree && n) root_cover_box(ctx);
    RtBvhInfo& bi = ctx->info;
    bi.triangles = n;
    bi.nodes = flat.nodes; bi.leaves = flat.leaves; bi.empty_leaves = flat.empty_leaves; bi.interior = flat.interior;
    bi.max_depth_reached = flat.max_depth_reached; bi.max_leaf_size = flat.max_leaf_size;
    bi.child_records = flat.n_records;
    bi.device_bytes = (flat.recs.size() + flat.tris.size() + flat.shade.size()) * sizeof(F4) + flat.orig.size() * sizeof(int32_t);
    bi.build_ms = t1 - t0 + wide_ms;
    bi.upload_ms = t2 - t1;
    ctx->bvh_valid = true;
    return RT_OK;
}

int rt_bvh_info(const RtContext* ctx, RtBvhInfo* out)
{
    if (!ctx || !out) return RT_ERR_INVALID;
    if (!ctx->bvh_valid) return RT_ERR_STATE;
    *out = ctx->info;
    return RT_OK;
}

int rt_transform_triangles(RtContext* ctx, const float m[16], int max_depth, int leaf_max_obj_count)
{
    if (!ctx || !m) return RT_ERR_INVALID;
    if (int r = bind(ctx)) return r;
    M4 t;
    memcpy(t.m, m, sizeof(t.m));
    ctx->bvh_valid = false;
    if (ctx->opt_device_build && ctx->db.tris_on_device && !ctx->xyz9.empty()) {
        devbuild::k_ob_transform<<<ctx->sm_count * 8, 256, 0, ctx->stream>>>(ctx->db.xyz9.p, ctx->xyz9.size() / 3, t);
        RT_CUDA(ctx, cudaGetLastError());
        ctx->db.host_pending.push_back(t);
    } else {
        apply_pending_host_transforms(ctx);
        transform_host_vertices(ctx, t);
        ctx->db.tris_on_device = false;
    }
    return rt_build_bvh(ctx, max_depth, leaf_max_obj_count);
}

int rt_set_materials(RtContext* ctx, const RtMaterial* mats, size_t n)
{
    if (!ctx) return RT_ERR_INVALID;
    if (int r = bind(ctx)) return r;
// ... 34 lines not shown
    ctx->shapes.push_back(make_plane(point, normal, mat_index));
    return upload_shapes(ctx);
}

int rt_clear_analytic_shapes(RtContext* ctx)
{
    if (!ctx) return RT_ERR_INVALID;
    ctx->shapes.clear();
    return RT_OK;
}

static int set_texture(RtContext* ctx, int slot, const void* data, int width, int height, int format)
{
    if (!ctx) return RT_ERR_INVALID;
    if (int r = bind(ctx)) return r;
    if (slot < 0 || slot >= RT_TEX_COUNT) return fail(ctx, RT_ERR_INVALID, "texture slot %d", slot);
    if (!data || width <= 0 || height <= 0) return fail(ctx, RT_ERR_INVALID, "texture %dx%d", width, height);
    RT_CUDA(ctx, cudaStreamSynchronize(ctx->stream));
    Texture& t = ctx->tex[slot];
    const size_t bytes = (size_t)width * height * (format == 1 ? 4 : 16);
    const size_t had = (size_t)t.w * t.h * (t.format == 1 ? 4 : 16);
    if (!t.d || had != bytes) {
        if (t.d) cudaFree(t.d);
        t = Texture();
        RT_CUDA(ctx, cudaMalloc(&t.d, bytes));
    }
    t.w = 0; t.h = 0; t.format = 0;
    RT_CUDA(ctx, cudaMemcpy(t.d, data, bytes, cudaMemcpyHostToDevice));
    t.w = width; t.h = height; t.format = format;
    return RT_OK;
}

int rt_set_texture_f32(RtContext* ctx, int slot, const float* rgba, int width, int height) { return set_texture(ctx, slot, rgba, width, height, 2); }
int rt_set_texture_u8(RtContext* ctx, int slot, const uint8_t* rgba, int width, int height) { return set_texture(ctx, slot, rgba, width, height, 1); }

int rt_clear_texture(RtContext* ctx, int slot)
{
    if (!ctx) return RT_ERR_INVALID;
    if (int r = bind(ctx)) return r;
    if (slot < 0 || slot >= RT_TEX_COUNT) return fail(ctx, RT_ERR_INVALID, "texture slot %d", slot);
    RT_CUDA(ctx, cudaStreamSynchronize(ctx->stream));
    if (ctx->tex[slot].d) cudaFree(ctx->tex[slot].d);
    ctx->tex[slot] = Texture();
    return RT_OK;
}

int rt_set_camera(RtContext* ctx, const float proj_inv[16], const float cam_to_world[16], const float position[3])
{
    if (!ctx || !proj_inv || !cam_to_world || !position) return RT_ERR_INVALID;
    memcpy(ctx->proj_inv.m, proj_inv, 64);
    memcpy(ctx->cam_to_world.m, cam_to_world, 64);
    ctx->cam_pos = v3(position[0], position[1], position[2]);
    ctx->camera_set = true;
    return RT_OK;
}

int rt_set_projection(RtContext* ctx, float fov, float aspect, float znear, float zfar)
{
    if (!ctx) return RT_ERR_INVALID;
    if (!(aspect > 0.0f) || !(zfar > znear)) return fail(ctx, RT_ERR_INVALID, "projection: aspect %g, znear %g, zfar %g", aspect, znear, zfar);
    ctx->proj = perspective_matrix(fov, aspect, znear, zfar);
    ctx->proj_fov = fov;
    ctx->proj_aspect = aspect;
    ctx->proj_set = true;
    return RT_OK;
}

int rt_set_light(RtContext* ctx, const float position[3])
{
    if (!ctx || !position) return RT_ERR_INVALID;
    ctx->light = v3(position[0], position[1], position[2]);
    return RT_OK;
}

int rt_screen_coverage(const float proj_inv[16], const float cam_to_world[16], const float position[3], int rw, int rh,
                       const float* boxes, size_t n_boxes, double margin_scale, uint32_t* bits, size_t n_words)
{
    if (!proj_inv || !cam_to_world || !position || rw <= 0 || rh <= 0 || (n_boxes && !boxes) || !bits) return RT_ERR_INVALID;
    M4 pinv, c2w;
    memcpy(pinv.m, proj_inv, 64);
    memcpy(c2w.m, cam_to_world, 64);
    std::vector<uint32_t> out;
    int32_t words = 0;
    const bool bound = screen_coverage(c2w, pinv, v3(position[0], position[1], position[2]), rw, rh, boxes, n_boxes, margin_scale, out, words);
    if (out.size() > n_words) return RT_ERR_INVALID;
    std::copy(out.begin(), out.end(), bits);
    return bound ? 1 : 0;
}

int rt_tile_count(const RtSettings* s, int tile_size, int tile_mod, int tile_rem)
{
    if (!s || tile_size <= 0 || tile_mod <= 0 || tile_rem < 0 || tile_rem >= tile_mod) return RT_ERR_INVALID;
    return (int)owned_tiles(s, tile_size, tile_mod, tile_rem, nullptr).size();
}

int rt_render_device_begin(RtContext* ctx, const RtSettings* s, uint32_t* d_argb_out, int tile_size, int tile_mod, int tile_rem)
{
    if (!ctx) return RT_ERR_INVALID;
    if (ctx->pending.active) return fail(ctx, RT_ERR_STATE, "rt_render_device_begin: the previous frame has not been ended (rt_render_device_end)");
    if (int r = bind(ctx)) return r;
    if (int r = validate_settings(ctx, s)) return r;
    if (int r = validate_scene_for_render(ctx, s)) return r;
    if (int r = check_tile_args(ctx, tile_size, tile_mod, tile_rem)) return r;
    if (!d_argb_out) return fail(ctx, RT_ERR_INVALID, "d_argb_out is NULL");
    const bool ssao = s->enable_ssao != 0;
    const bool raster = s->hybrid_rasterization_tracing != 0;
    if (raster && tile_mod != 1) return fail(ctx, RT_ERR_UNSUPPORTED, "hybrid_rasterization_tracing renders the whole frame on one GPU (one z-buffer)");
    if (raster && !ctx->proj_set) return fail(ctx, RT_ERR_STATE, "hybrid_rasterization_tracing: the projection has not been set (rt_set_projection)");
    if (ssao && tile_mod != 1) return fail(ctx, RT_ERR_UNSUPPORTED, "enable_ssao needs the whole frame on one GPU: its samples read the z-buffer of neighbouring tiles");
    if (ssao && !ctx->proj_set) return fail(ctx, RT_ERR_STATE, "enable_ssao: the projection has not been set (rt_set_projection)");

    bool rebuild_masks = false;
    if (ctx->tune.packets && s->compute_shadows && s->shading_method == RT_SHADING)
        if (int r = plan_light_masks(ctx, rebuild_masks)) return r;
    const FrameView fr = frame_view(ctx, s);
    const SceneView sc = scene_view(ctx);
    const SceneView scp = packet_view(ctx);
    const bool resolve = fr.factor > 1;
    const bool reflect = ctx->any_reflective && s->shading_method == RT_SHADING;
    if (reflect) if (int r = ensure_stack(ctx, s)) return r;

    TileList* tl = nullptr;
    if (int r = get_tile_list(ctx, s, tile_size, tile_mod, tile_rem, &tl)) return r;
    const std::vector<uint32_t>& owned = tl->host;
    const int tiles_x = tl->tiles_x;
    WorkView wk = {};
    wk.tiles_x = tiles_x;
    wk.tile_px = tile_size * fr.factor;
    wk.patches_per_side = (wk.tile_px + kPatch - 1) / kPatch;
    const bool has_shapes = !ctx->shapes.empty();
    const bool cull = ctx->opt_screen_cull && ctx->tune.packets && !has_shapes && !raster;
    if (cull) if (int r = update_cover(ctx, fr)) return r;
    wk.cover = (cull && ctx->cover_bound) ? ctx->d_cover.p : nullptr;
    wk.cover_words = wk.cover ? ctx->cover_words : 0;
    const bool classify = wk.cover != nullptr && tl->count > 0;
    if (classify) {
        if (!tl->split_valid || tl->split_cover != ctx->cover_generation || tl->split_tile_px != wk.tile_px) {
            std::vector<uint32_t> in, out;
            for (uint32_t tile : owned) {
                const int x0 = (int)(tile % (uint32_t)tiles_x) * wk.tile_px, y0 = (int)(tile / (uint32_t)tiles_x) * wk.tile_px;
                const int x1 = std::min(x0 + wk.tile_px, fr.rw) - 1, y1 = std::min(y0 + wk.tile_px, fr.rh) - 1;
                const bool hit = cover_any(ctx->h_cover, ctx->cover_words, x0, y0, x1, y1);
                (hit ? in : out).push_back(tile);
            }
            tl->n_traced = (uint32_t)in.size();
            tl->split_host = in;
            tl->split_host.insert(tl->split_host.end(), out.begin(), out.end());
            if (!tl->d_split) RT_CUDA(ctx, cudaMalloc((void**)&tl->d_split, tl->count * sizeof(uint32_t)));
            RT_CUDA(ctx, cudaStreamSynchronize(ctx->stream));
            RT_CUDA(ctx, cudaMemcpy(tl->d_split, tl->split_host.data(), tl->count * sizeof(uint32_t), cudaMemcpyHostToDevice));
            tl->split_cover = ctx->cover_generation;
            tl->split_tile_px = wk.tile_px;
            tl->split_valid = true;
        }
    }
    const uint32_t n_traced = raster ? 0u : (classify ? tl->n_traced : tl->count);
    const std::vector<uint32_t> tiles(classify ? tl->split_host.begin() : owned.begin(), (classify ? tl->split_host.begin() : owned.begin()) + n_traced);
    const uint64_t px_per_tile = (uint64_t)wk.patches_per_side * wk.patches_per_side * kPatch * kPatch;
    uint32_t tiles_per_chunk = (uint32_t)std::max<uint64_t>(1, ctx->opt_chunk_pixels / px_per_tile);
    if ((tiles.size() + tiles_per_chunk - 1) / tiles_per_chunk > (size_t)kMaxChunks)
        tiles_per_chunk = (uint32_t)((tiles.size() + kMaxChunks - 1) / kMaxChunks);
    const int n_lanes = (ctx->opt_lanes > 1 && tune_packets_hint(ctx)) ? (int)std::min<size_t>((size_t)ctx->opt_lanes, std::max<size_t>(tiles.size(), 1)) : 1;
    if (n_lanes > 1 && tiles.size() <= (size_t)tiles_per_chunk * (n_lanes - 1)) tiles_per_chunk = (uint32_t)((tiles.size() + n_lanes - 1) / n_lanes);
    std::vector<uint32_t> bounds;
    for (size_t b = 0; b < tiles.size(); b += tiles_per_chunk) bounds.push_back((uint32_t)b);
    bounds.push_back((uint32_t)tiles.size());
    const uint32_t n_chunks = (uint32_t)bounds.size() - 1u;
    uint32_t largest_chunk = 0;
    for (uint32_t c = 0; c < n_chunks; c++) largest_chunk = std::max(largest_chunk, bounds[c + 1] - bounds[c]);
    const size_t qcap = (size_t)largest_chunk * px_per_tile;

    RT_CUDA(ctx, ctx->d_counters.ensure(std::max<uint32_t>(n_chunks, 1)));
    const int pw = grid_for(ctx, (const void*)k_primary_packet<false, false>, kPrimaryThreads) * (kPrimaryThreads / 32);
    const bool short_launch = (uint64_t)owned.size() * px_per_tile / 32 < (uint64_t)256 * (uint64_t)pw;
    auto largest = [](int32_t v) { return v >= 0 ? v : std::min<int32_t>(-v, 1 << 27) * 8; };
    auto least = [](int32_t v, int div) { return v >= 0 ? 0 : std::max<int32_t>(1, -v / div); };
    Tuning tune = ctx->tune;
    tune.packet_rounds = largest(ctx->tune.packet_rounds); tune.packet_min = least(ctx->tune.packet_rounds, 4);
    tune.item_rounds = largest(ctx->tune.item_rounds); tune.item_min = least(ctx->tune.item_rounds, 1);
    tune.primary_rounds = largest(ctx->tune.primary_rounds); tune.primary_min = least(ctx->tune.primary_rounds, 4);
    if (ctx->tune.primary_rounds < 0 && !short_launch) tune.primary_rounds = tune.primary_min = 0;
    if (tune.fused && tune.packets) {
        auto magnitude = [](int32_t v) { return v >= 0 ? v : -v; };
        tune.packet_rounds = magnitude(ctx->tune.packet_rounds);
        tune.item_rounds = magnitude(ctx->tune.item_rounds);
        tune.primary_rounds = magnitude(ctx->tune.primary_rounds);
        tune.packet_min = tune.item_min = tune.primary_min = 0;
    }
    const bool tail = tune.packets && tune.packet_rounds > 0 && s->compute_shadows && s->shading_method == RT_SHADING;
    const bool psplit = tune.packets && tune.primary_rounds > 0;
    const bool sort_hits = ctx->opt_shadow_sort && tune.packets && !tune.fused && !reflect && s->compute_shadows && s->shading_method == RT_SHADING &&
                           !(ctx->opt_shadow_sort == 2 && tl->last_hit_fraction >= 0.3f);
    LightMap light_map;
    memset(&light_map, 0, sizeof(light_map));
    if (sort_hits) light_map = make_light_map(ctx);
    const size_t split_cap = (tail || psplit) ? std::min<size_t>(std::max<size_t>(qcap / 32, 1024), (size_t)1 << 20) : 0;
    const size_t item_cap = (tail || psplit) ? std::min<size_t>(std::max<size_t>(qcap / 4, (size_t)1 << 14), (size_t)1 << 21) : 0;
    for (int l = 0; l < n_lanes; l++) {
        QueueSet& Q = ctx->qs[l];
        if (tail || psplit) {
            RT_CUDA(ctx, Q.split_base.ensure(split_cap)); RT_CUDA(ctx, Q.split_active.ensure(split_cap)); RT_CUDA(ctx, Q.split_occ.ensure(split_cap));
            RT_CUDA(ctx, Q.items.ensure(item_cap * kItemPasses));
            if (tune.fused) {
                if (Q.item_ready.n < item_cap * kItemPasses) {
                    RT_CUDA(ctx, Q.item_ready.ensure(item_cap * kItemPasses));
                    RT_CUDA(ctx, cudaMemsetAsync(Q.item_ready.p, 0, Q.item_ready.n * sizeof(uint32_t), ctx->stream));
                }
                RT_CUDA(ctx, Q.split_pending.ensure(split_cap));
            }
        }
        if (psplit) RT_CUDA(ctx, Q.split_best.ensure(split_cap * 32));
        RT_CUDA(ctx, Q.hit_slot.ensure(qcap)); RT_CUDA(ctx, Q.tri.ensure(qcap)); RT_CUDA(ctx, Q.t.ensure(qcap));
        RT_CUDA(ctx, Q.u.ensure(qcap)); RT_CUDA(ctx, Q.v.ensure(qcap));
        if (reflect) { RT_CUDA(ctx, Q.refl_idx.ensure(qcap)); RT_CUDA(ctx, Q.refl_rgb.ensure(3 * qcap)); RT_CUDA(ctx, Q.refl_cnt.ensure(3 * qcap)); }
        if (sort_hits) {
            RT_CUDA(ctx, Q.hit_sorted.ensure(qcap)); RT_CUDA(ctx, Q.sort_keys.ensure(qcap));
            RT_CUDA(ctx, Q.sort_bins.ensure((size_t)kSortBins + kSortScanBlocks));
// ... 718 lines not shown
```

Measured before the change: 25080.

## Start primary packet traversal from per-block screen-space BVH entry cuts

Adds per-camera entry cuts: for each 8x4 pixel block, a device kernel projects upper wide-tree node boxes to screen rectangles and greedily expands the root into up to eight nodes whose projections reach the block. Primary packet traversal then seeds its stack from these cut nodes instead of testing the root and upper levels. This is meant to skip top-level box tests and node fetches for primary rays. It adds per-frame cut kernels and memory, plus an extra ballot/shuffle per packet, and requires all lanes of a warp to fall in one block.

```diff
diff --git a/include/rtb200.h b/include/rtb200.h
--- a/include/rtb200.h
+++ b/include/rtb200.h
@@ -150,6 +150,7 @@
     RT_OPT_GRAPH = 18,
     RT_OPT_RASTER_UNITS = 17,
     RT_OPT_LIGHT_CULL = 21,
+    RT_OPT_ENTRY_CUTS = 22,
     RT_OPT_LEAF_SPLIT = 2
 };
 int rt_set_option(RtContext* ctx, int option, int64_t value);
diff --git a/raytracercpp_b200/api.py b/raytracercpp_b200/api.py
--- a/raytracercpp_b200/api.py
+++ b/raytracercpp_b200/api.py
@@ -15,7 +15,7 @@
 RT_TEX_DISPLACEMENT = 11
 RT_OPT_COUNT_WORK, RT_OPT_CHUNK_PIXELS, RT_OPT_LEAF_SPLIT, RT_OPT_REFILL_PRIMARY, RT_OPT_REFILL_SHADE, RT_OPT_TRI_BATCH, RT_OPT_PACKETS = 0, 1, 2, 3, 4, 5, 6
 RT_OPT_PACKET_ROUNDS, RT_OPT_SCREEN_CULL, RT_OPT_LANES, RT_OPT_ITEM_ROUNDS, RT_OPT_PRIMARY_ROUNDS, RT_OPT_FUSED_ITEMS, RT_OPT_TOP_TABLE, RT_OPT_SHADOW_SORT, RT_OPT_DEVICE_BUILD, RT_OPT_ITEM_PASSES = 7, 8, 9, 10, 11, 12, 13, 14, 15, 16
-RT_OPT_RASTER_UNITS, RT_OPT_GRAPH, RT_OPT_PACKET_CULL, RT_OPT_FAN_LANES, RT_OPT_LIGHT_CULL = 17, 18, 19, 20, 21
+RT_OPT_RASTER_UNITS, RT_OPT_GRAPH, RT_OPT_PACKET_CULL, RT_OPT_FAN_LANES, RT_OPT_LIGHT_CULL, RT_OPT_ENTRY_CUTS = 17, 18, 19, 20, 21, 22
 
 
 class RtError(RuntimeError):
diff --git a/raytracercpp_b200/build.py b/raytracercpp_b200/build.py
--- a/raytracercpp_b200/build.py
+++ b/raytracercpp_b200/build.py
@@ -10,7 +10,7 @@
 CSRC = PKG / "csrc"
 LIB = PKG / "librtb200.so"
 SOURCES = [CSRC / "rtb200.cu", CSRC / "octree_build.cpp", CSRC / "scene_io.cpp"]
-HEADERS = [CSRC / "kernels.cuh", CSRC / "octree_device.cuh", CSRC / "light_cull.cuh", CSRC / "host_common.h", CSRC / "rt_device.h", CSRC / "rt_math.h", CSRC / "scene_layout.h",
+HEADERS = [CSRC / "kernels.cuh", CSRC / "octree_device.cuh", CSRC / "light_cull.cuh", CSRC / "entry_cuts.cuh", CSRC / "host_common.h", CSRC / "rt_device.h", CSRC / "rt_math.h", CSRC / "scene_layout.h",
            CSRC / "ssao.cuh", CSRC / "ssao_device.h", CSRC / "raster.cuh", CSRC / "raster_device.h",
            PKG.parent / "include" / "rtb200.h"]
 
diff --git a/raytracercpp_b200/csrc/entry_cuts.cuh b/raytracercpp_b200/csrc/entry_cuts.cuh
--- /dev/null
+++ b/raytracercpp_b200/csrc/entry_cuts.cuh
@@ -0,0 +1,143 @@
+#pragma once
+
+#include "rt_device.h"
+
+namespace rtb {
+namespace entrycut {
+
+constexpr uint32_t kCutSlots = 8;
+
+struct CutRect {
+    int32_t x0, y0, x1, y1;
+};
+
+struct CutNode {
+    uint32_t pos;
+    uint32_t first;
+    uint32_t kids;
+    float area;
+};
+
+struct CoverCamera {
+    int rw, rh, bw, bh;
+    double w2c[16], proj[16], pos[3];
+    double pos_max, e_dir, dc, lmin, margin_scale;
+};
+
+RT_HD CutRect box_blocks(const CoverCamera& cc, const float* bx)
+{
+    const double eps = 0x1p-24;
+    const double kTriRel = 0x1p-14;
+    const double ndc_slack = 1e-9;
+    const CutRect none = {1, 1, 0, 0}, all = {0, 0, cc.bw - 1, cc.bh - 1};
+    const double* pos = cc.pos;
+    bool finite = true, empty = false;
+    double lo[3], hi[3], bmax = 0.0;
+    for (int k = 0; k < 3; k++) {
+        lo[k] = bx[k]; hi[k] = bx[3 + k];
+        finite &= isfinite(lo[k]) && isfinite(hi[k]);
+        empty |= lo[k] > hi[k];
+        bmax = fmax(bmax, fmax(fabs(lo[k]), fabs(hi[k])));
+    }
+    if (empty) return none;
+    if (!finite) return all;
+    double sfar = 0.0;
+    for (int c = 0; c < 8; c++) {
+        double d2 = 0.0;
+        for (int k = 0; k < 3; k++) { const double x = ((c >> k) & 1 ? hi[k] : lo[k]) - pos[k]; d2 += x * x; }
+        sfar = fmax(sfar, sqrt(d2));
+    }
+    const double e_tri = kTriRel * (cc.pos_max + bmax + sfar);
+    const double reach = (sfar + e_tri) * (1.0 + 5.0 * eps);
+    const double r = cc.margin_scale * (e_tri + reach * cc.e_dir + cc.dc * (2.0 + reach / cc.lmin));
+    double xmin = 1e300, xmax = -1e300, ymin = 1e300, ymax = -1e300;
+    for (int c = 0; c < 8; c++) {
+        const double p[4] = {(c & 1 ? hi[0] + r : lo[0] - r), (c & 2 ? hi[1] + r : lo[1] - r), (c & 4 ? hi[2] + r : lo[2] - r), 1.0};
+        double vv[4], cl[4];
+        for (int i = 0; i < 4; i++) vv[i] = cc.w2c[4 * i] * p[0] + cc.w2c[4 * i + 1] * p[1] + cc.w2c[4 * i + 2] * p[2] + cc.w2c[4 * i + 3] * p[3];
+        if (!(fabs(vv[3]) > 1e-12)) return all;
+        for (int i = 0; i < 3; i++) vv[i] /= vv[3];
+        vv[3] = 1.0;
+        for (int i = 0; i < 4; i++) cl[i] = cc.proj[4 * i] * vv[0] + cc.proj[4 * i + 1] * vv[1] + cc.proj[4 * i + 2] * vv[2] + cc.proj[4 * i + 3] * vv[3];
+        if (!(cl[3] > 1e-3 * (1.0 + fabs(vv[2])))) return all;
+        const double nx = cl[0] / cl[3], ny = cl[1] / cl[3];
+        if (!isfinite(nx) || !isfinite(ny)) return all;
+        xmin = fmin(xmin, nx); xmax = fmax(xmax, nx); ymin = fmin(ymin, ny); ymax = fmax(ymax, ny);
+    }
+    const double lim = 1e9;
+    const double px0 = ceil(fmax(-lim, (xmin - ndc_slack + 1.0) * 0.5 * cc.rw - 0.5)), px1 = floor(fmin(lim, (xmax + ndc_slack + 1.0) * 0.5 * cc.rw - 0.5));
+    const double py0 = ceil(fmax(-lim, (ymin - ndc_slack + 1.0) * 0.5 * cc.rh - 0.5)), py1 = floor(fmin(lim, (ymax + ndc_slack + 1.0) * 0.5 * cc.rh - 0.5));
+    const int x0 = (int)fmax(0.0, px0), x1 = (int)fmin((double)cc.rw - 1, px1);
+    const int y0 = (int)fmax(0.0, py0), y1 = (int)fmin((double)cc.rh - 1, py1);
+    if (x0 > x1 || y0 > y1) return none;
+    return CutRect{x0 >> 3, y0 >> 2, x1 >> 3, y1 >> 2};
+}
+
+RT_HD bool cut_reaches(const CutRect& r, int32_t bx, int32_t by) { return bx >= r.x0 && bx <= r.x1 && by >= r.y0 && by <= r.y1; }
+
+RT_HD int entry_cut(const CutRect* rect, const CutNode* node, uint32_t n_expand, int32_t bx, int32_t by, uint32_t m[kCutSlots])
+{
+    if (n_expand == 0u || node[0].kids == 0u) return 0;
+    constexpr uint32_t kKeep = 0xffffffffu;
+    uint32_t reach[kCutSlots];
+    float area[kCutSlots];
+    int n = 0;
+    auto put = [&](int at, uint32_t i) {
+        m[at] = i;
+        const bool expand = i < n_expand && node[i].kids != 0u;
+        uint32_t c = 0;
+        for (uint32_t k = 0; expand && k < node[i].kids; k++) c += cut_reaches(rect[node[i].first + k], bx, by) ? 1u : 0u;
+        reach[at] = expand ? c : kKeep;
+        area[at] = expand ? node[i].area : 0.0f;
+    };
+    for (uint32_t k = 0; k < node[0].kids; k++)
+        if (cut_reaches(rect[node[0].first + k], bx, by)) put(n++, node[0].first + k);
+    for (;;) {
+        int best = -1;
+        for (int k = 0; k < n; k++)
+            if (reach[k] != kKeep && n - 1 + (int)reach[k] <= (int)kCutSlots && (best < 0 || area[k] > area[best])) best = k;
+        if (best < 0) break;
+        const uint32_t i = m[best];
+        const int c = (int)reach[best];
+        if (c == 0) {
+            for (int k = best; k + 1 < n; k++) { m[k] = m[k + 1]; reach[k] = reach[k + 1]; area[k] = area[k + 1]; }
+            n--;
+            continue;
+        }
+        for (int k = n - 1; k > best; k--) {
+            m[k + c - 1] = m[k]; reach[k + c - 1] = reach[k]; area[k + c - 1] = area[k];
+        }
+        int at = best;
+        for (uint32_t k = 0; k < node[i].kids; k++)
+            if (cut_reaches(rect[node[i].first + k], bx, by)) put(at++, node[i].first + k);
+        n += c - 1;
+    }
+    return n;
+}
+
+#ifdef __CUDACC__
+__global__ void __launch_bounds__(128)
+k_cut_rects(CoverCamera cc, const float* boxes, uint32_t n, CutRect* rect)
+{
+    const uint32_t i = blockIdx.x * blockDim.x + threadIdx.x;
+    if (i < n) rect[i] = box_blocks(cc, boxes + 6 * (size_t)i);
+}
+
+__global__ void __launch_bounds__(256)
+k_entry_cuts(const CutRect* rect, const CutNode* node, uint32_t n_expand, const uint32_t* cover, int32_t cover_words, int32_t bw, int32_t bh,
+             uint4* cuts)
+{
+    const uint32_t b = blockIdx.x * blockDim.x + threadIdx.x;
+    if (b >= (uint32_t)bw * (uint32_t)bh) return;
+    const int32_t bx = (int32_t)(b % (uint32_t)bw), by = (int32_t)(b / (uint32_t)bw);
+    if (!((cover[(size_t)by * cover_words + (bx >> 5)] >> (bx & 31)) & 1u)) return;
+    uint32_t m[kCutSlots], pos[kCutSlots];
+    const int n = entry_cut(rect, node, n_expand, bx, by, m);
+    for (int k = 0; k < (int)kCutSlots; k++) pos[k] = k < n ? node[m[k]].pos : 0u;
+    cuts[2 * (size_t)b] = make_uint4(pos[0], pos[1], pos[2], pos[3]);
+    cuts[2 * (size_t)b + 1] = make_uint4(pos[4], pos[5], pos[6], pos[7]);
+}
+#endif
+
+}
+}
diff --git a/raytracercpp_b200/csrc/kernels.cuh b/raytracercpp_b200/csrc/kernels.cuh
--- a/raytracercpp_b200/csrc/kernels.cuh
+++ b/raytracercpp_b200/csrc/kernels.cuh
@@ -9,6 +9,7 @@
 constexpr int kPrimaryThreads = 128;
 constexpr int kQueueThreads = 128;
 constexpr int kPrimaryFetch = 1;
+constexpr uint32_t kMetaStaged = 0x20000000u;
 constexpr int kStepsPerCheck = 4;
 constexpr unsigned kParkCtas = 296;
 constexpr unsigned kFusedGenerations = 12;
@@ -92,7 +93,19 @@
     int32_t patches_per_side;
     const uint32_t* cover;
     int32_t cover_words;
+    const uint4* cuts;
 };
+
+RT_DEV const uint32_t* packet_cut(const WorkView& wk, const FrameView& fr, bool active, int px, int py)
+{
+    if (wk.cuts == nullptr) return nullptr;
+    const unsigned am = __ballot_sync(0xffffffffu, active);
+    if (am == 0u) return nullptr;
+    const int lead = __ffs(am) - 1;
+    const int bx = __shfl_sync(0xffffffffu, px >> 3, lead), by = __shfl_sync(0xffffffffu, py >> 2, lead);
+    if (__ballot_sync(0xffffffffu, active && ((px >> 3) != bx || (py >> 2) != by)) != 0u) return nullptr;
+    return reinterpret_cast<const uint32_t*>(wk.cuts + 2 * ((size_t)by * (size_t)((fr.rw + 7) >> 3) + (size_t)bx));
+}
 
 struct QueueView {
     int32_t* slot_tri;
@@ -400,7 +413,8 @@
 RT_DEV bool packet_trace(const SceneView& sc, PacketStack& K, const float4* top, bool& active, V3 o, V3 d, float t_max, V3 p, float dist2,
                          HitRec& best, bool& occluded, TraceCounters& tc, unsigned& overflow, int max_rounds, unsigned& rounds,
                          uint32_t start_link = 0u, uint32_t start_meta = 0u, int32_t best_orig = 0x7fffffff,
-                         const unsigned int* poll_occ = nullptr, const unsigned long long* poll_best = nullptr, Drain drain = no_drain())
+                         const unsigned int* poll_occ = nullptr, const unsigned long long* poll_best = nullptr, Drain drain = no_drain(),
+                         const uint32_t* cut = nullptr)
 {
     const unsigned lane = threadIdx.x & 31u;
     SlabRay sr;
@@ -425,7 +439,22 @@
     const bool swap_lo = ordered && ((neg_mask >> (2u * f)) & 1u) != 0u;
     const bool swap_hi = ordered && f < 3u && ((neg_mask >> (2u * f + 1u)) & 1u) != 0u;
     uint32_t link = start_link, meta = start_meta;
-    if (start_meta == 0u) {
+    uint32_t cut_pos = 0u;
+    unsigned cut_lanes = 0u;
+    if (!ANY && start_meta == 0u && cut != nullptr) {
+        cut_pos = __ldg(cut + (lane >> 2));
+        cut_lanes = __ballot_sync(0xffffffffu, cut_pos != 0u);
+    }
+    if (cut_lanes != 0u) {
+        if (cut_pos != 0u) {
+            float4 v = RT_LDG4(sc.recs + 4 * (size_t)cut_pos + (lane & 3u));
+            if (swap_lo) { const float t = v.x; v.x = v.y; v.y = t; }
+            if (swap_hi) { const float t = v.z; v.z = v.w; v.w = t; }
+            K.stage[lane] = v;
+        }
+        link = 0u;
+        meta = kMetaStaged | ((uint32_t)__popc(cut_lanes) >> 2);
+    } else if (start_meta == 0u) {
         const rt_f4* r = sc.recs;
         rt_f4 q0 = RT_LDG4(r), q1 = RT_LDG4(r + 1), q2 = RT_LDG4(r + 2), q3 = RT_LDG4(r + 3);
         if (COUNT && active) tc.vol_tests++;
@@ -471,7 +500,7 @@
         if (!(meta & RT_LEAF_BIT)) {
             const uint32_t count = meta & RT_META_COUNT_MASK;
             const bool in_top = top != nullptr && (meta & RT_META_TOP) != 0u;
-            if (lane < 4u * count) {
+            if (lane < 4u * count && !(meta & kMetaStaged)) {
                 float4 v = in_top ? top[4u * ((meta >> RT_META_TOP_SHIFT) & 0xffu) + lane] : RT_LDG4(sc.recs + 4 * (size_t)link + lane);
                 if (swap_lo) { const float t = v.x; v.x = v.y; v.y = t; }
                 if (swap_hi) { const float t = v.z; v.z = v.w; v.w = t; }
@@ -634,6 +663,7 @@
                 }
                 continue;
             }
+            const uint32_t* cut = packet_cut(wk, fr, active, px, py);
             if (active) primary_ray(fr, px, py, o, d);
             traced += (uint32_t)__popc(__ballot_sync(0xffffffffu, active));
             HitRec best;
@@ -642,7 +672,7 @@
             const unsigned long long t0 = COUNT ? global_ns() : 0ull;
             if (!((tune.cull & 1) != 0 && packet_set_cull(K, active, o, o + d, 0.0f))) packet_no_cull(K);
             const bool finished = packet_trace<false, COUNT, true>(sc, K, top, live, o, d, INFINITY, o, 0.0f, best, occ, tc, overflow, tune.primary_rounds, rounds,
-                                                                   0u, 0u, 0x7fffffff, nullptr, nullptr, make_drain(&cnt->next_patch, total, tune.primary_min));
+                                                                   0u, 0u, 0x7fffffff, nullptr, nullptr, make_drain(&cnt->next_patch, total, tune.primary_min), cut);
             __syncwarp();
             if (COUNT && lane == 0) note_packet(cnt, 0, rounds, global_ns() - t0);
             if (!finished) {
@@ -1836,6 +1866,7 @@
                 super[(size_t)py * fr.rw + px] = quantise_argb(shade_miss(sc, fr, d));
             }
         } else {
+            const uint32_t* cut = packet_cut(wk, fr, active, px, py);
             if (active) primary_ray(fr, px, py, o, d);
             traced += (uint32_t)__popc(__ballot_sync(0xffffffffu, active));
             HitRec best;
@@ -1843,7 +1874,8 @@
             unsigned rounds = 0;
             const unsigned long long t0 = COUNT ? global_ns() : 0ull;
             const bool finished = packet_trace<false, COUNT>(sc, K, top, live, o, d, INFINITY, o, 0.0f, best, occ, tc, overflow,
-                                                             fq_budget(tune.primary_rounds, rem), rounds);
+                                                             fq_budget(tune.primary_rounds, rem), rounds, 0u, 0u, 0x7fffffff, nullptr, nullptr,
+                                                             no_drain(), cut);
             __syncwarp();
             if (COUNT && lane == 0) note_packet(cnt, 0, rounds, global_ns() - t0);
             if (!finished) {
diff --git a/raytracercpp_b200/csrc/octree_device.cuh b/raytracercpp_b200/csrc/octree_device.cuh
--- a/raytracercpp_b200/csrc/octree_device.cuh
+++ b/raytracercpp_b200/csrc/octree_device.cuh
@@ -1,6 +1,7 @@
 #pragma once
 
 #include "scene_layout.h"
+#include "entry_cuts.cuh"
 
 namespace rtb {
 namespace devbuild {
@@ -623,15 +624,21 @@
 }
 
 __global__ void __launch_bounds__(256)
-k_wb_boxes(const float4* recs, const uint32_t* src, const uint32_t* info, uint32_t n, uint32_t first_kept, float* boxes)
+k_wb_upper(const float4* recs, const uint32_t* src, Cells C, uint32_t n, float* boxes, entrycut::CutNode* nodes)
 {
     const uint32_t node = blockIdx.x * blockDim.x + threadIdx.x;
     if (node >= n) return;
     const float4 q0 = recs[4 * (size_t)src[node]], q1 = recs[4 * (size_t)src[node] + 1];
-    const bool keep = node >= first_kept || (info[node] & 15u) == 0u;
     float* b = boxes + 6 * (size_t)node;
-    b[0] = keep ? q0.x : INFINITY; b[1] = keep ? q0.z : INFINITY; b[2] = keep ? q1.x : INFINITY;
-    b[3] = keep ? q0.y : -INFINITY; b[4] = keep ? q0.w : -INFINITY; b[5] = keep ? q1.y : -INFINITY;
+    b[0] = q0.x; b[1] = q0.z; b[2] = q1.x;
+    b[3] = q0.y; b[4] = q0.w; b[5] = q1.y;
+    const uint32_t kids = C.info[node] & 15u;
+    entrycut::CutNode c;
+    c.pos = C.rec[node];
+    c.first = kids ? C.first_child[node] : 0u;
+    c.kids = kids;
+    c.area = kids ? wb_axis_area(recs, src[node]) : 0.0f;
+    nodes[node] = c;
 }
 
 __global__ void __launch_bounds__(256)
diff --git a/raytracercpp_b200/csrc/rtb200.cu b/raytracercpp_b200/csrc/rtb200.cu
--- a/raytracercpp_b200/csrc/rtb200.cu
+++ b/raytracercpp_b200/csrc/rtb200.cu
@@ -21,6 +21,7 @@
 #include "scene_layout.h"
 #include "octree_device.cuh"
 #include "light_cull.cuh"
+#include "entry_cuts.cuh"
 #include "ssao.cuh"
 #include "raster.cuh"
 #include "host_common.h"
@@ -32,6 +33,7 @@
 constexpr uint64_t kChunkPixels = 1ull << 28;
 constexpr int kMaxChunks = 256;
 constexpr uint32_t kCoverBoxes = 4096;
+constexpr uint32_t kCutNodes = 65536;
 
 thread_local std::string g_create_error;
 std::atomic<unsigned long long> g_alloc_generation{0};
@@ -227,13 +229,21 @@
     bool proj_set = false;
     float root_lo[3] = {0, 0, 0}, root_hi[3] = {0, 0, 0};
     std::vector<float> cover_boxes;
-    struct CoverInputs { M4 proj_inv, cam_to_world; V3 cam_pos; int32_t rw, rh; uint64_t tree; } cover_in{};
+    std::vector<uint8_t> cover_set;
+    struct CoverInputs { M4 proj_inv, cam_to_world; V3 cam_pos; int32_t rw, rh; uint64_t tree; uint32_t cuts; } cover_in{};
     bool cover_valid = false;
     bool cover_bound = false;
     int32_t cover_words = 0;
     std::vector<uint32_t> h_cover;
     DevBuf<uint32_t> d_cover;
     uint64_t cover_generation = 0;
+    bool opt_entry_cuts = true;
+    uint32_t cut_expand = 0;
+    DevBuf<entrycut::CutNode> d_cut_nodes;
+    DevBuf<entrycut::CutRect> d_cut_rects;
+    DevBuf<uint4> d_cuts;
+    std::vector<entrycut::CutNode> h_cut_nodes;
+    bool cuts_built = false;
 
     bool opt_light_cull = true;
     DevBuf<uint32_t> d_tri_occ, d_blk_occ, d_rec_parent;
@@ -476,22 +486,10 @@
     return true;
 }
 
-bool screen_coverage(const M4& cam_to_world, const M4& proj_inv, V3 cam_pos, int rw, int rh, const float* boxes, size_t n_boxes,
-                     double margin_scale, std::vector<uint32_t>& bits, int32_t& words_per_row)
-{
-    const int bw = (rw + 7) / 8, bh = (rh + 3) / 4;
-    words_per_row = (bw + 31) / 32;
-    bits.assign((size_t)words_per_row * (size_t)bh, 0u);
-    auto set_blocks = [&](int bx0, int by0, int bx1, int by1) {
-        for (int by = by0; by <= by1; by++) {
-            uint32_t* row = bits.data() + (size_t)by * words_per_row;
-            for (int w = bx0 >> 5; w <= bx1 >> 5; w++) {
-                const int lo = std::max(bx0 - 32 * w, 0), hi = std::min(bx1 - 32 * w, 31);
-                row[w] |= (hi == 31 ? 0xffffffffu : ((1u << (hi + 1)) - 1u)) & ~((1u << lo) - 1u);
-            }
-        }
-    };
-    if (n_boxes == 0) return true;
+bool cover_camera(const M4& cam_to_world, const M4& proj_inv, V3 cam_pos, int rw, int rh, double margin_scale, entrycut::CoverCamera& cc)
+{
+    cc.rw = rw; cc.rh = rh; cc.bw = (rw + 7) / 8; cc.bh = (rh + 3) / 4;
+    cc.margin_scale = margin_scale;
     double c2w[16], pinv[16], w2c[16], proj[16];
     for (int i = 0; i < 16; i++) { c2w[i] = (&cam_to_world.m[0][0])[i]; pinv[i] = (&proj_inv.m[0][0])[i]; }
     if (!invert4(c2w, w2c) || !invert4(pinv, proj)) return false;
@@ -562,54 +560,41 @@
     const double nn = std::sqrt(n[0] * n[0] + n[1] * n[1] + n[2] * n[2]);
     const double lmin = std::fabs(n[0] * (ws_c[0][0] - pos[0]) + n[1] * (ws_c[0][1] - pos[1]) + n[2] * (ws_c[0][2] - pos[2])) / nn;
     if (!(lmin > 4.0 * e3n)) return false;
-    const double e_dir = 2.0 * e3n / lmin + 5.0 * eps;
-    const double kTriRel = 0x1p-14;
-    const double pos_max = std::max(std::fabs(pos[0]), std::max(std::fabs(pos[1]), std::fabs(pos[2])));
-    const double ndc_slack = 1e-9;
+    cc.e_dir = 2.0 * e3n / lmin + 5.0 * eps;
+    cc.pos_max = std::max(std::fabs(pos[0]), std::max(std::fabs(pos[1]), std::fabs(pos[2])));
+    cc.dc = dc;
+    cc.lmin = lmin;
+    for (int i = 0; i < 16; i++) { cc.w2c[i] = w2c[i]; cc.proj[i] = proj[i]; }
+    for (int k = 0; k < 3; k++) cc.pos[k] = pos[k];
+    return true;
+}
+
+bool screen_coverage(const M4& cam_to_world, const M4& proj_inv, V3 cam_pos, int rw, int rh, const float* boxes, size_t n_boxes,
+                     const uint8_t* in_set, double margin_scale, std::vector<uint32_t>& bits, int32_t& words_per_row,
+                     std::vector<entrycut::CutRect>* rects = nullptr)
+{
+    const int bw = (rw + 7) / 8, bh = (rh + 3) / 4;
+    words_per_row = (bw + 31) / 32;
+    bits.assign((size_t)words_per_row * (size_t)bh, 0u);
+    if (rects) rects->clear();
+    if (n_boxes == 0) return true;
+    entrycut::CoverCamera cc;
+    if (!cover_camera(cam_to_world, proj_inv, cam_pos, rw, rh, margin_scale, cc)) return false;
+    std::vector<entrycut::CutRect> local;
+    std::vector<entrycut::CutRect>& rr = rects ? *rects : local;
+    rr.resize(n_boxes);
+#pragma omp parallel for schedule(static) if (n_boxes > 4096)
+    for (long long b = 0; b < (long long)n_boxes; b++) rr[b] = entrycut::box_blocks(cc, boxes + 6 * b);
     for (size_t b = 0; b < n_boxes; b++) {
-        const float* bx = boxes + 6 * b;
-        bool finite = true, empty = false;
-        double lo[3], hi[3], bmax = 0.0;
-        for (int k = 0; k < 3; k++) {
-            lo[k] = bx[k]; hi[k] = bx[3 + k];
-            finite &= std::isfinite(lo[k]) && std::isfinite(hi[k]);
-            empty |= lo[k] > hi[k];
-            bmax = std::max(bmax, std::max(std::fabs(lo[k]), std::fabs(hi[k])));
-        }
-        if (empty) continue;
-        if (!finite) { set_blocks(0, 0, bw - 1, bh - 1); return true; }
-        double sfar = 0.0;
-        for (int c = 0; c < 8; c++) {
-            double d2 = 0.0;
-            for (int k = 0; k < 3; k++) { const double x = ((c >> k) & 1 ? hi[k] : lo[k]) - pos[k]; d2 += x * x; }
-            sfar = std::max(sfar, std::sqrt(d2));
-        }
-        const double e_tri = kTriRel * (pos_max + bmax + sfar);
-        const double reach = (sfar + e_tri) * (1.0 + 5.0 * eps);
-        const double r = margin_scale * (e_tri + reach * e_dir + dc * (2.0 + reach / lmin));
-        double xmin = 1e300, xmax = -1e300, ymin = 1e300, ymax = -1e300;
-        bool whole = false;
-        for (int c = 0; c < 8 && !whole; c++) {
-            const double p[4] = {(c & 1 ? hi[0] + r : lo[0] - r), (c & 2 ? hi[1] + r : lo[1] - r), (c & 4 ? hi[2] + r : lo[2] - r), 1.0};
-            double vv[4], cc[4];
-            for (int i = 0; i < 4; i++) vv[i] = w2c[4 * i] * p[0] + w2c[4 * i + 1] * p[1] + w2c[4 * i + 2] * p[2] + w2c[4 * i + 3] * p[3];
-            if (!(std::fabs(vv[3]) > 1e-12)) { whole = true; break; }
-            for (int i = 0; i < 3; i++) vv[i] /= vv[3];
-            vv[3] = 1.0;
-            for (int i = 0; i < 4; i++) cc[i] = proj[4 * i] * vv[0] + proj[4 * i + 1] * vv[1] + proj[4 * i + 2] * vv[2] + proj[4 * i + 3] * vv[3];
-            if (!(cc[3] > 1e-3 * (1.0 + std::fabs(vv[2])))) { whole = true; break; }
-            const double nx = cc[0] / cc[3], ny = cc[1] / cc[3];
-            if (!std::isfinite(nx) || !std::isfinite(ny)) { whole = true; break; }
-            xmin = std::min(xmin, nx); xmax = std::max(xmax, nx); ymin = std::min(ymin, ny); ymax = std::max(ymax, ny);
-        }
-        if (whole) { set_blocks(0, 0, bw - 1, bh - 1); return true; }
-        const double lim = 1e9;
-        const double px0 = std::ceil(std::max(-lim, (xmin - ndc_slack + 1.0) * 0.5 * rw - 0.5)), px1 = std::floor(std::min(lim, (xmax + ndc_slack + 1.0) * 0.5 * rw - 0.5));
-        const double py0 = std::ceil(std::max(-lim, (ymin - ndc_slack + 1.0) * 0.5 * rh - 0.5)), py1 = std::floor(std::min(lim, (ymax + ndc_slack + 1.0) * 0.5 * rh - 0.5));
-        const int x0 = (int)std::max(0.0, px0), x1 = (int)std::min((double)rw - 1, px1);
-        const int y0 = (int)std::max(0.0, py0), y1 = (int)std::min((double)rh - 1, py1);
-        if (x0 > x1 || y0 > y1) continue;
-        set_blocks(x0 >> 3, y0 >> 2, x1 >> 3, y1 >> 2);
+        const entrycut::CutRect& r = rr[b];
+        if ((in_set && !in_set[b]) || r.x0 > r.x1) continue;
+        for (int by = r.y0; by <= r.y1; by++) {
+            uint32_t* row = bits.data() + (size_t)by * words_per_row;
+            for (int w = r.x0 >> 5; w <= r.x1 >> 5; w++) {
+                const int lo = std::max(r.x0 - 32 * w, 0), hi = std::min(r.x1 - 32 * w, 31);
+                row[w] |= (hi == 31 ? 0xffffffffu : ((1u << (hi + 1)) - 1u)) & ~((1u << lo) - 1u);
+            }
+        }
     }
     return true;
 }
@@ -633,26 +618,66 @@
     memset(&in, 0, sizeof(in));
     in.proj_inv = ctx->proj_inv; in.cam_to_world = ctx->cam_to_world; in.cam_pos = ctx->cam_pos;
     in.rw = fr.rw; in.rh = fr.rh; in.tree = ctx->tree_serial;
+    in.cuts = ctx->opt_entry_cuts && ctx->cut_expand > 0 ? 1u : 0u;
     if (ctx->cover_valid && memcmp(&in, &ctx->cover_in, sizeof(in)) == 0) return RT_OK;
     ctx->cover_valid = false;
+    ctx->cuts_built = false;
+    static const bool trace = getenv("RTB200_TRACE") != nullptr;
+    const size_t n_boxes = ctx->cover_boxes.size() / 6, n_set = ctx->cover_set.empty() ? n_boxes : ctx->cover_set.size();
     const double t0 = now_ms();
-    ctx->cover_bound = screen_coverage(ctx->cam_to_world, ctx->proj_inv, ctx->cam_pos, fr.rw, fr.rh, ctx->cover_boxes.data(),
-                                       ctx->cover_boxes.size() / 6, 1.0, ctx->h_cover, ctx->cover_words);
+    ctx->cover_bound = screen_coverage(ctx->cam_to_world, ctx->proj_inv, ctx->cam_pos, fr.rw, fr.rh, ctx->cover_boxes.data(), n_set,
+                                       ctx->cover_set.empty() ? nullptr : ctx->cover_set.data(), 1.0, ctx->h_cover, ctx->cover_words);
     const double t1 = now_ms();
-    double t2 = t1;
+    double t2 = t1, t3 = t1;
+    const int32_t bw = (fr.rw + 7) / 8, bh = (fr.rh + 3) / 4;
     if (ctx->cover_bound) {
         RT_CUDA(ctx, cudaStreamSynchronize(ctx->stream));
         t2 = now_ms();
         RT_CUDA(ctx, ctx->d_cover.ensure(ctx->h_cover.size()));
         RT_CUDA(ctx, cudaMemcpyAsync(ctx->d_cover.p, ctx->h_cover.data(), ctx->h_cover.size() * sizeof(uint32_t), cudaMemcpyHostToDevice, ctx->stream));
-    }
-    static const bool trace = getenv("RTB200_TRACE") != nullptr;
+        entrycut::CoverCamera cc;
+        if (in.cuts && cover_camera(ctx->cam_to_world, ctx->proj_inv, ctx->cam_pos, fr.rw, fr.rh, 1.0, cc)) {
+            const size_t n_blocks = (size_t)bw * (size_t)bh;
+            RT_CUDA(ctx, ctx->d_cut_rects.ensure(n_boxes));
+            RT_CUDA(ctx, ctx->d_cuts.ensure(2 * n_blocks));
+            if (trace) { RT_CUDA(ctx, cudaStreamSynchronize(ctx->stream)); t3 = now_ms(); }
+            entrycut::k_cut_rects<<<(unsigned)((n_boxes + 127) / 128), 128, 0, ctx->stream>>>(cc, ctx->db.w_boxes.p, (uint32_t)n_boxes, ctx->d_cut_rects.p);
+            entrycut::k_entry_cuts<<<(unsigned)((n_blocks + 255) / 256), 256, 0, ctx->stream>>>(ctx->d_cut_rects.p, ctx->d_cut_nodes.p, ctx->cut_expand,
+                                                                                           ctx->d_cover.p, ctx->cover_words, bw, bh, ctx->d_cuts.p);
+            RT_CUDA(ctx, cudaGetLastError());
+            ctx->cuts_built = true;
+        }
+    }
     if (trace) {
+        RT_CUDA(ctx, cudaStreamSynchronize(ctx->stream));
+        const double t4 = now_ms();
         size_t set = 0;
         for (uint32_t w : ctx->h_cover) set += (size_t)__builtin_popcount(w);
-        const size_t blocks = (size_t)((fr.rw + 7) / 8) * (size_t)((fr.rh + 3) / 4);
-        fprintf(stderr, "[rtb200] screen coverage: %zu boxes, bound %d, %.4f of the blocks covered, build %.3f ms, upload %.3f ms\n",
-                ctx->cover_boxes.size() / 6, (int)ctx->cover_bound, ctx->cover_bound ? (double)set / (double)blocks : 1.0, t1 - t0, now_ms() - t2);
+        const size_t blocks = (size_t)bw * (size_t)bh;
+        const size_t in_set = ctx->cover_set.empty() ? n_boxes : (size_t)std::count(ctx->cover_set.begin(), ctx->cover_set.end(), (uint8_t)1);
+        fprintf(stderr, "[rtb200] screen coverage: %zu boxes (%zu in the bitmap's set), bound %d, %.4f of the blocks covered, build %.3f ms, upload %.3f ms\n",
+                n_boxes, in_set, (int)ctx->cover_bound, ctx->cover_bound ? (double)set / (double)blocks : 1.0, t1 - t0, (ctx->cuts_built ? t3 : t4) - t2);
+        if (ctx->cuts_built) {
+            std::vector<entrycut::CutRect> rects(n_boxes);
+            RT_CUDA(ctx, cudaMemcpy(rects.data(), ctx->d_cut_rects.p, n_boxes * sizeof(entrycut::CutRect), cudaMemcpyDeviceToHost));
+            std::vector<uint32_t> level(n_boxes, 0u);
+            for (size_t i = 0; i < n_boxes; i++)
+                for (uint32_t k = 0; k < ctx->h_cut_nodes[i].kids && i < ctx->cut_expand; k++) level[ctx->h_cut_nodes[i].first + k] = level[i] + 1u;
+            double members = 0.0, depth = 0.0;
+            size_t with = 0;
+            for (int32_t by = 0; by < bh; by++)
+                for (int32_t bx = 0; bx < bw; bx++) {
+                    if (!((ctx->h_cover[(size_t)by * ctx->cover_words + (bx >> 5)] >> (bx & 31)) & 1u)) continue;
+                    uint32_t m[entrycut::kCutSlots];
+                    const int n = entrycut::entry_cut(rects.data(), ctx->h_cut_nodes.data(), ctx->cut_expand, bx, by, m);
+                    if (n == 0) continue;
+                    with++;
+                    members += n;
+                    for (int k = 0; k < n; k++) depth += level[m[k]];
+                }
+            fprintf(stderr, "[rtb200] entry cuts: %zu nodes (levels below node %u expand), %zu of %zu covered blocks have a cut, %.2f members, mean level %.2f, "
+                    "build %.3f ms\n", n_boxes, ctx->cut_expand, with, set, with ? members / (double)with : 0.0, members > 0 ? depth / members : 0.0, t4 - t3);
+        }
     }
     ctx->cover_in = in;
     ctx->cover_valid = true;
@@ -763,6 +788,8 @@
 void root_cover_box(RtContext* ctx)
 {
     ctx->cover_boxes.assign({ctx->root_lo[0], ctx->root_lo[1], ctx->root_lo[2], ctx->root_hi[0], ctx->root_hi[1], ctx->root_hi[2]});
+    ctx->cover_set.clear();
+    ctx->cut_expand = 0;
 }
 
 int build_wide_tree(RtContext* ctx, uint64_t n_records)
@@ -801,16 +828,6 @@
         level_first.push_back(lf + lc); level_count.push_back(total);
     }
     const uint32_t n_nodes = level_first.back() + level_count.back();
-    {
-        size_t lv = 0;
-        while (lv + 1 < level_first.size() && level_count[lv + 1] <= kCoverBoxes) lv++;
-        const uint32_t n_box = level_first[lv] + level_count[lv];
-        RT_CUDA(ctx, D.w_boxes.ensure(6 * (size_t)n_box));
-        k_wb_boxes<<<(n_box + 255) / 256, 256, 0, st>>>(recs, D.w_src.p, C.info, n_box, level_first[lv], D.w_boxes.p);
-        ctx->cover_boxes.resize(6 * (size_t)n_box);
-        RT_CUDA(ctx, cudaMemcpyAsync(ctx->cover_boxes.data(), D.w_boxes.p, 6 * (size_t)n_box * sizeof(float), cudaMemcpyDeviceToHost, st));
-        RT_CUDA(ctx, cudaStreamSynchronize(st));
-    }
     for (int l = (int)level_first.size() - 1; l >= 0; l--)
         k_wb_size<<<(level_count[l] + 255) / 256, 256, 0, st>>>(C, level_first[l], level_count[l]);
     uint32_t root_size = 0;
@@ -825,6 +842,28 @@
     for (size_t l = 0; l < level_first.size(); l++)
         k_ob_place<<<(level_count[l] + 255) / 256, 256, 0, st>>>(C, level_first[l], level_count[l], P);
     k_wb_records<<<(n_nodes + 255) / 256, 256, 0, st>>>(recs, D.w_src.p, C, n_nodes, (float4*)ctx->d_wrecs.p);
+    {
+        size_t lb = 0, lv = 0;
+        while (lb + 1 < level_first.size() && level_count[lb + 1] <= kCoverBoxes) lb++;
+        while (lv + 1 < level_first.size() && (uint64_t)level_first[lv + 1] + level_count[lv + 1] <= kCutNodes) lv++;
+        const size_t last = std::max(lb, lv);
+        const uint32_t n_box = level_first[last] + level_count[last];
+        RT_CUDA(ctx, D.w_boxes.ensure(6 * (size_t)n_box));
+        RT_CUDA(ctx, ctx->d_cut_nodes.ensure(n_box));
+        k_wb_upper<<<(n_box + 255) / 256, 256, 0, st>>>(recs, D.w_src.p, C, n_box, D.w_boxes.p, ctx->d_cut_nodes.p);
+        ctx->cover_boxes.resize(6 * (size_t)n_box);
+        ctx->h_cut_nodes.resize(n_box);
+        RT_CUDA(ctx, cudaMemcpyAsync(ctx->cover_boxes.data(), D.w_boxes.p, 6 * (size_t)n_box * sizeof(float), cudaMemcpyDeviceToHost, st));
+        RT_CUDA(ctx, cudaMemcpyAsync(ctx->h_cut_nodes.data(), ctx->d_cut_nodes.p, n_box * sizeof(entrycut::CutNode), cudaMemcpyDeviceToHost, st));
+        RT_CUDA(ctx, cudaStreamSynchronize(st));
+        const uint32_t b_first = level_first[lb], b_end = level_first[lb] + level_count[lb];
+        ctx->cover_set.resize(b_end);
+        for (uint32_t i = 0; i < b_end; i++) ctx->cover_set[i] = i >= b_first || ctx->h_cut_nodes[i].kids == 0u;
+        ctx->cut_expand = level_first[lv];
+        if (getenv("RTB200_TRACE"))
+            fprintf(stderr, "[rtb200] upper levels: bitmap level B = %zu (%u nodes, %u boxes in the set), cut level D = %zu (%u nodes), %u nodes in all\n",
+                    lb, level_count[lb], b_end, lv, level_count[lv], n_box);
+    }
     k_ob_top_table<<<1, 32, 0, st>>>((float4*)ctx->d_wrecs.p, (float4*)ctx->d_top.p, D.stats.p);
     uint32_t top_n = 0;
     RT_CUDA(ctx, cudaMemcpyAsync(&top_n, &D.stats.p->top_n, 4, cudaMemcpyDeviceToHost, st));
@@ -1084,6 +1123,7 @@
     if (ctx->lane_fork) cudaEventDestroy(ctx->lane_fork);
     for (auto e : ctx->lane_join) if (e) cudaEventDestroy(e);
     ctx->d_counters.release(); ctx->d_flag.release();
+    ctx->d_cut_nodes.release(); ctx->d_cut_rects.release(); ctx->d_cuts.release();
     ctx->b_a.release(); ctx->b_b.release(); ctx->b_t.release(); ctx->b_u.release(); ctx->b_v.release(); ctx->b_id.release(); ctx->b_occ.release();
     if (ctx->pending.host_cnt) cudaFreeHost(ctx->pending.host_cnt);
     if (ctx->h_frame) cudaFreeHost(ctx->h_frame);
@@ -1147,6 +1187,7 @@
         return RT_OK;
     case RT_OPT_GRAPH: ctx->opt_graph = value != 0; return RT_OK;
     case RT_OPT_LIGHT_CULL: ctx->opt_light_cull = value != 0; return RT_OK;
+    case RT_OPT_ENTRY_CUTS: ctx->opt_entry_cuts = value != 0; return RT_OK;
     case RT_OPT_FAN_LANES: ctx->opt_fan_lanes = value != 0; return RT_OK;
     case RT_OPT_PACKET_CULL:
         if (value < 0 || value > 3) return fail(ctx, RT_ERR_INVALID, "packet cull %lld outside [0,3]", (long long)value);
@@ -1202,6 +1243,8 @@
     ctx->bvh_valid = false;
     ctx->wide_tree = false;
     ctx->cover_boxes.clear();
+    ctx->cover_set.clear();
+    ctx->cut_expand = 0;
     ctx->tree_serial++;
     if (ctx->opt_device_build && n > 0) return build_bvh_device(ctx, max_depth, leaf_max_obj_count);
     apply_pending_host_transforms(ctx);
@@ -1402,10 +1445,42 @@
     memcpy(c2w.m, cam_to_world, 64);
     std::vector<uint32_t> out;
     int32_t words = 0;
-    const bool bound = screen_coverage(c2w, pinv, v3(position[0], position[1], position[2]), rw, rh, boxes, n_boxes, margin_scale, out, words);
+    const bool bound = screen_coverage(c2w, pinv, v3(position[0], position[1], position[2]), rw, rh, boxes, n_boxes, nullptr, margin_scale, out, words);
     if (out.size() > n_words) return RT_ERR_INVALID;
     std::copy(out.begin(), out.end(), bits);
     return bound ? 1 : 0;
+}
+
+int rt_entry_cuts(const float proj_inv[16], const float cam_to_world[16], const float position[3], int rw, int rh, const float* boxes,
+                  const uint32_t* first, const uint32_t* kids, size_t n_nodes, uint32_t n_expand, double margin_scale, uint32_t* cuts, size_t n_cuts)
+{
+    if (!proj_inv || !cam_to_world || !position || rw <= 0 || rh <= 0 || n_nodes == 0 || !boxes || !first || !kids || !cuts || n_expand > n_nodes)
+        return RT_ERR_INVALID;
+    const int32_t bw = (rw + 7) / 8, bh = (rh + 3) / 4;
+    if (n_cuts < entrycut::kCutSlots * (size_t)bw * (size_t)bh) return RT_ERR_INVALID;
+    std::vector<entrycut::CutNode> nodes(n_nodes);
+    for (size_t i = 0; i < n_nodes; i++) {
+        if (kids[i] > 8u || (i < n_expand && kids[i] && (first[i] <= i || (size_t)first[i] + kids[i] > n_nodes))) return RT_ERR_INVALID;
+        const float* b = boxes + 6 * i;
+        const float dx = b[3] - b[0], dy = b[4] - b[1], dz = b[5] - b[2];
+        nodes[i] = entrycut::CutNode{(uint32_t)i, first[i], kids[i], dx * dy + dy * dz + dz * dx};
+    }
+    M4 pinv, c2w;
+    memcpy(pinv.m, proj_inv, 64);
+    memcpy(c2w.m, cam_to_world, 64);
+    std::vector<uint32_t> bits;
+    std::vector<entrycut::CutRect> rects;
+    int32_t words = 0;
+    if (!screen_coverage(c2w, pinv, v3(position[0], position[1], position[2]), rw, rh, boxes, n_nodes, nullptr, margin_scale, bits, words, &rects))
+        return 0;
+    for (int32_t by = 0; by < bh; by++)
+        for (int32_t bx = 0; bx < bw; bx++) {
+            uint32_t* out = cuts + entrycut::kCutSlots * ((size_t)by * bw + bx);
+            uint32_t m[entrycut::kCutSlots];
+            const int n = entrycut::entry_cut(rects.data(), nodes.data(), n_expand, bx, by, m);
+            for (int k = 0; k < (int)entrycut::kCutSlots; k++) out[k] = k < n ? m[k] : 0u;
+        }
+    return 1;
 }
 
 int rt_tile_count(const RtSettings* s, int tile_size, int tile_mod, int tile_rem)
@@ -1453,6 +1528,7 @@
     if (cull) if (int r = update_cover(ctx, fr)) return r;
     wk.cover = (cull && ctx->cover_bound) ? ctx->d_cover.p : nullptr;
     wk.cover_words = wk.cover ? ctx->cover_words : 0;
+    wk.cuts = (wk.cover != nullptr && ctx->cuts_built) ? ctx->d_cuts.p : nullptr;
     const bool classify = wk.cover != nullptr && tl->count > 0;
     if (classify) {
         if (!tl->split_valid || tl->split_cover != ctx->cover_generation || tl->split_tile_px != wk.tile_px) {
```

Result: faster. 26080, median of 6 (+4.0%).
